# CIawevy/FreeFine

Measured on NVIDIA B200. Metric: edits/s @512^2 50-step SD1.5 (FreeFine 2-D geometric edit), higher is better.
Workload: dtype bf16

## Files before the change

### freefine_b200/csrc/attn_tcgen05.cu

```cuda
#include <cuda.h>
#include <cuda_bf16.h>

#include <atomic>
#include <cstdlib>
#include <type_traits>

#include "ff_common.cuh"

namespace {

constexpr int BM = 128;
constexpr int BN = 64;
constexpr int BOX_COLS = 64;
constexpr int TILE_BYTES = BM * 128;
constexpr int KV_BYTES = BN * 128;
constexpr int NUM_SOFTMAX_WARPS = 8;
constexpr int NUM_THREADS = 32 * (NUM_SOFTMAX_WARPS + 2);
template <bool HILO> constexpr float rescale_threshold() { return HILO ? 24.f : 8.f; }
#ifndef FF_RING_DEFAULT
#define FF_RING_DEFAULT 6
#endif
#ifndef FF_POLY_PATTERN
#define FF_POLY_PATTERN 0x92
#endif
#ifndef FF_T32_DEFAULT
#define FF_T32_DEFAULT 0
#endif
#ifndef FF_SEP_P
#define FF_SEP_P 0
#endif
#ifndef FF_SELF_ISSUE
#define FF_SELF_ISSUE 0
#endif

template <int DPAD, bool HILO> struct Cfg {
  static constexpr int DPV = DPAD == 16 ? 16 : (DPAD == 48 ? 48 : DPAD + 16);
  static constexpr int NKT = (DPAD + BOX_COLS - 1) / BOX_COLS;
  static_assert((DPV + BOX_COLS - 1) / BOX_COLS == NKT, "V tile must span as many boxes as the K tile");
  static constexpr int NSTAGE = DPAD <= 48 ? 4 : (DPAD <= 80 ? 3 : 2);
  static_assert(NSTAGE >= 2, "QK(t+1) is issued before PV(t): tile t+1 must fit beside tile t");
  static constexpr bool SEP = FF_SEP_P && DPAD == 48 && !HILO && NSTAGE == 4;
  static constexpr int TMEM_S = 0, TMEM_P = 2 * BN, TMEM_O = 2 * BN + (SEP ? BN / 2 : 0);
  static constexpr int TMEM_USED = TMEM_O + 2 * DPV;
  static constexpr int TMEM_COLS = TMEM_USED <= 256 ? 256 : 512;
  static constexpr int SMEM_Q = NKT * TILE_BYTES;
  static constexpr int SMEM_STAGE = 2 * NKT * KV_BYTES;
  static constexpr int ACC_LD = DPAD <= 80 ? DPAD + 4 : DPAD;
  static constexpr int SMEM_ACC = BM * ACC_LD * 4;
  static constexpr int SMEM_MX = 2 * BM * 4;
  static constexpr int SMEM_BYTES = SMEM_Q + NSTAGE * SMEM_STAGE + SMEM_ACC + SMEM_MX + 1024  + 256 ;
  static_assert(SMEM_BYTES <= 227 * 1024, "shared memory budget");
  static constexpr int MIN_CTAS = (SMEM_BYTES <= 113 * 1024 && TMEM_COLS == 256) ? 2 : 1;
  static constexpr bool SELF = FF_SELF_ISSUE && !SEP && DPAD == 48 && !HILO && NSTAGE == 4;
  static constexpr int THREADS = SELF ? 32 * (NUM_SOFTMAX_WARPS + 1) : NUM_THREADS;
};

__device__ __forceinline__ uint32_t smem_u32(const void* p) { return (uint32_t)__cvta_generic_to_shared(p); }

__device__ __forceinline__ void mbar_init(uint32_t bar, uint32_t count) {
  asm volatile("mbarrier.init.shared::cta.b64 [%0], %1;" ::"r"(bar), "r"(count));
}
__device__ __forceinline__ void mbar_expect_tx(uint32_t bar, uint32_t bytes) {
  asm volatile("mbarrier.arrive.expect_tx.shared::cta.b64 _, [%0], %1;" ::"r"(bar), "r"(bytes) : "memory");
}
__device__ __forceinline__ void mbar_arrive(uint32_t bar) {
  asm volatile("mbarrier.arrive.shared::cta.b64 _, [%0];" ::"r"(bar) : "memory");
}
__device__ __forceinline__ uint32_t mbar_try(uint32_t bar, uint32_t parity) {
  uint32_t done;
#ifdef FF_TRYWAIT_NOHINT
  asm volatile(
      "{\n\t.reg .pred p;\n\t"
      "mbarrier.try_wait.parity.shared::cta.b64 p, [%1], %2;\n\t"
      "selp.u32 %0, 1, 0, p;\n\t}"
      : "=r"(done)
      : "r"(bar), "r"(parity)
      : "memory");
#else
  asm volatile(
      "{\n\t.reg .pred p;\n\t"
      "mbarrier.try_wait.parity.shared::cta.b64 p, [%1], %2, %3;\n\t"
      "selp.u32 %0, 1, 0, p;\n\t}"
      : "=r"(done)
      : "r"(bar), "r"(parity), "r"(0x989680u)
      : "memory");
#endif
  return done;
}
__device__ __forceinline__ bool mbar_test(uint32_t bar, uint32_t parity) {
  uint32_t done;
  asm volatile(
      "{\n\t.reg .pred p;\n\t"
      "mbarrier.test_wait.parity.shared::cta.b64 p, [%1], %2;\n\t"
      "selp.u32 %0, 1, 0, p;\n\t}"
      : "=r"(done)
      : "r"(bar), "r"(parity)
      : "memory");
  return done != 0;
}
#ifndef FF_WAIT_FORM
#define FF_WAIT_FORM 1
#endif
__device__ __noinline__ void mbar_wait_slow(uint32_t bar, uint32_t parity) {
#if FF_WAIT_FORM == 0
  const long long t0 = clock64();
  while (!mbar_try(bar, parity)) {
    if (clock64() - t0 > 4000000000LL) {
      printf("ff_attn: mbarrier wait timed out (block %d,%d,%d thread %d bar %u parity %u)\n", blockIdx.x,
             blockIdx.y, blockIdx.z, threadIdx.x, bar, parity);
      __trap();
    }
  }
#else
  const long long t0 = clock64();
#pragma unroll 1
  for (uint32_t n = 1;; ++n) {
    if ((n & 15u) == 0 && clock64() - t0 > 4000000000LL) break;
#if FF_WAIT_FORM == 1
    if (mbar_try(bar, parity)) return;
#else
    uint32_t done;
    asm volatile(
        "{\n\t.reg .pred p;\n\t"
        "mbarrier.try_wait.parity.shared::cta.b64 p, [%1], %2;\n\t"
        "selp.u32 %0, 1, 0, p;\n\t}"
        : "=r"(done)
        : "r"(bar), "r"(parity)
        : "memory");
    if (done) return;
#endif
  }
  printf("ff_attn: mbarrier wait timed out (block %d,%d,%d thread %d bar %u parity %u)\n", blockIdx.x, blockIdx.y,
         blockIdx.z, threadIdx.x, bar, parity);
  __trap();
#endif
}
__device__ __forceinline__ void mbar_wait(uint32_t bar, uint32_t parity) {
  if (!mbar_try(bar, parity)) mbar_wait_slow(bar, parity);
}
#ifndef FF_SPIN_MASK
#define FF_SPIN_MASK 0
#endif
template <int ROLE_BIT>
__device__ __forceinline__ void mbar_wait_hot(uint32_t bar, uint32_t parity) {
  if constexpr ((FF_SPIN_MASK >> ROLE_BIT) & 1) {
    for (uint32_t n = 0; !mbar_test(bar, parity); ++n) {
#ifdef FF_SPIN_SLEEP
      __nanosleep(FF_SPIN_SLEEP);
#endif
      if (n > (1u << 24)) { mbar_wait_slow(bar, parity); return; }
    }
  } else {
    mbar_wait(bar, parity);
  }
}
__device__ __forceinline__ void tma_load_4d(uint32_t dst, const CUtensorMap* map, int c0, int c1, int c2, int c3,
                                            uint32_t bar) {
  asm volatile(
      "cp.async.bulk.tensor.4d.shared::cluster.global.tile.mbarrier::complete_tx::bytes [%0], [%1, {%2, %3, %4, %5}], [%6];"
      ::"r"(dst), "l"(map), "r"(c0), "r"(c1), "r"(c2), "r"(c3), "r"(bar)
      : "memory");
}
__device__ __forceinline__ void named_bar_sync(int id, int count) {
  switch (id) {
    case 1: asm volatile("bar.sync 1, %0;" ::"r"(count) : "memory"); break;
    case 2: asm volatile("bar.sync 2, %0;" ::"r"(count) : "memory"); break;
    case 3: asm volatile("bar.sync 3, %0;" ::"r"(count) : "memory"); break;
    default: asm volatile("bar.sync 4, %0;" ::"r"(count) : "memory"); break;
  }
}
__device__ __forceinline__ bool elect_one() {
  uint32_t pred;
  asm volatile("{\n\t.reg .pred p;\n\telect.sync _|p, 0xffffffff;\n\tselp.u32 %0, 1, 0, p;\n\t}" : "=r"(pred));
  return pred != 0;
}
__device__ __forceinline__ void tc_fence_before() { asm volatile("tcgen05.fence::before_thread_sync;" ::: "memory"); }
__device__ __forceinline__ void tc_fence_after() { asm volatile("tcgen05.fence::after_thread_sync;" ::: "memory"); }
__device__ __forceinline__ void tc_commit(uint32_t bar) {
  asm volatile("tcgen05.commit.cta_group::1.mbarrier::arrive::one.shared::cluster.b64 [%0];" ::"r"(bar) : "memory");
}
__device__ __forceinline__ void mma_ss(uint32_t d_tmem, uint64_t a_desc, uint64_t b_desc, uint32_t idesc,
                                       uint32_t accumulate) {
  asm volatile(
      "{\n\t.reg .pred p;\n\tsetp.ne.b32 p, %4, 0;\n\t"
      "tcgen05.mma.cta_group::1.kind::f16 [%0], %1, %2, %3, p;\n\t}"
      ::"r"(d_tmem), "l"(a_desc), "l"(b_desc), "r"(idesc), "r"(accumulate)
      : "memory");
}
__device__ __forceinline__ void mma_ts(uint32_t d_tmem, uint32_t a_tmem, uint64_t b_desc, uint32_t idesc,
                                       uint32_t accumulate) {
  asm volatile(
      "{\n\t.reg .pred p;\n\tsetp.ne.b32 p, %4, 0;\n\t"
      "tcgen05.mma.cta_group::1.kind::f16 [%0], [%1], %2, %3, p;\n\t}"
      ::"r"(d_tmem), "r"(a_tmem), "l"(b_desc), "r"(idesc), "r"(accumulate)
      : "memory");
}
__device__ __forceinline__ void tmem_ld32(uint32_t taddr, float (&v)[32]) {
  uint32_t* r = reinterpret_cast<uint32_t*>(v);
  asm volatile(
      "tcgen05.ld.sync.aligned.32x32b.x32.b32 "
      "{%0, %1, %2, %3, %4, %5, %6, %7, %8, %9, %10, %11, %12, %13, %14, %15, "
      "%16, %17, %18, %19, %20, %21, %22, %23, %24, %25, %26, %27, %28, %29, %30, %31}, [%32];"
      : "=r"(r[0]), "=r"(r[1]), "=r"(r[2]), "=r"(r[3]), "=r"(r[4]), "=r"(r[5]), "=r"(r[6]), "=r"(r[7]),
        "=r"(r[8]), "=r"(r[9]), "=r"(r[10]), "=r"(r[11]), "=r"(r[12]), "=r"(r[13]), "=r"(r[14]), "=r"(r[15]),
        "=r"(r[16]), "=r"(r[17]), "=r"(r[18]), "=r"(r[19]), "=r"(r[20]), "=r"(r[21]), "=r"(r[22]), "=r"(r[23]),
        "=r"(r[24]), "=r"(r[25]), "=r"(r[26]), "=r"(r[27]), "=r"(r[28]), "=r"(r[29]), "=r"(r[30]), "=r"(r[31])
      : "r"(taddr)
      : "memory");
}
__device__ __forceinline__ void tmem_ld16(uint32_t taddr, float (&v)[16]) {
  uint32_t* r = reinterpret_cast<uint32_t*>(v);
  asm volatile(
      "tcgen05.ld.sync.aligned.32x32b.x16.b32 "
      "{%0, %1, %2, %3, %4, %5, %6, %7, %8, %9, %10, %11, %12, %13, %14, %15}, [%16];"
      : "=r"(r[0]), "=r"(r[1]), "=r"(r[2]), "=r"(r[3]), "=r"(r[4]), "=r"(r[5]), "=r"(r[6]), "=r"(r[7]),
        "=r"(r[8]), "=r"(r[9]), "=r"(r[10]), "=r"(r[11]), "=r"(r[12]), "=r"(r[13]), "=r"(r[14]), "=r"(r[15])
      : "r"(taddr)
      : "memory");
}
__device__ __forceinline__ float tmem_ld1_wait(uint32_t taddr) {
  uint32_t r;
  asm volatile("tcgen05.ld.sync.aligned.32x32b.x1.b32 {%0}, [%1];\n\ttcgen05.wait::ld.sync.aligned;"
               : "=r"(r) : "r"(taddr) : "memory");
  return __uint_as_float(r);
}
__device__ __forceinline__ void tmem_st16(uint32_t taddr, const uint32_t (&r)[16]) {
  asm volatile(
      "tcgen05.st.sync.aligned.32x32b.x16.b32 [%0], "
      "{%1, %2, %3, %4, %5, %6, %7, %8, %9, %10, %11, %12, %13, %14, %15, %16};"
      ::"r"(taddr), "r"(r[0]), "r"(r[1]), "r"(r[2]), "r"(r[3]), "r"(r[4]), "r"(r[5]), "r"(r[6]), "r"(r[7]),
        "r"(r[8]), "r"(r[9]), "r"(r[10]), "r"(r[11]), "r"(r[12]), "r"(r[13]), "r"(r[14]), "r"(r[15])
      : "memory");
}
__device__ __forceinline__ void tmem_wait_ld() { asm volatile("tcgen05.wait::ld.sync.aligned;" ::: "memory"); }
__device__ __forceinline__ void tmem_wait_ld16(float (&v)[16]) {
#ifdef FF_PLAIN_WAIT
  tmem_wait_ld();
  return;
#endif
  uint32_t* r = reinterpret_cast<uint32_t*>(v);
  asm volatile("tcgen05.wait::ld.sync.aligned;"
               : "+r"(r[0]), "+r"(r[1]), "+r"(r[2]), "+r"(r[3]), "+r"(r[4]), "+r"(r[5]), "+r"(r[6]), "+r"(r[7]),
                 "+r"(r[8]), "+r"(r[9]), "+r"(r[10]), "+r"(r[11]), "+r"(r[12]), "+r"(r[13]), "+r"(r[14]), "+r"(r[15])
               :
               : "memory");
}
__device__ __forceinline__ void tmem_wait_ld32(float (&v)[32]) {
#ifdef FF_PLAIN_WAIT
  tmem_wait_ld();
  return;
#endif
  uint32_t* r = reinterpret_cast<uint32_t*>(v);
  asm volatile("tcgen05.wait::ld.sync.aligned;"
               : "+r"(r[0]), "+r"(r[1]), "+r"(r[2]), "+r"(r[3]), "+r"(r[4]), "+r"(r[5]), "+r"(r[6]), "+r"(r[7]),
                 "+r"(r[8]), "+r"(r[9]), "+r"(r[10]), "+r"(r[11]), "+r"(r[12]), "+r"(r[13]), "+r"(r[14]), "+r"(r[15]),
                 "+r"(r[16]), "+r"(r[17]), "+r"(r[18]), "+r"(r[19]), "+r"(r[20]), "+r"(r[21]), "+r"(r[22]), "+r"(r[23]),
                 "+r"(r[24]), "+r"(r[25]), "+r"(r[26]), "+r"(r[27]), "+r"(r[28]), "+r"(r[29]), "+r"(r[30]), "+r"(r[31])
               :
               : "memory");
}
__device__ __forceinline__ void tmem_wait_st() { asm volatile("tcgen05.wait::st.sync.aligned;" ::: "memory"); }
__device__ __forceinline__ float fast_exp2(float x) {
#ifdef FF_KO_MUFU
  return x;
#else
  float y;
  asm("ex2.approx.ftz.f32 %0, %1;" : "=f"(y) : "f"(x));
  return y;
#endif
}

__device__ __forceinline__ uint64_t smem_desc_sw128(uint32_t saddr, uint32_t lbo_bytes) {
  return (uint64_t)((saddr & 0x3FFFFu) >> 4) | ((uint64_t)(lbo_bytes >> 4) << 16) | ((uint64_t)(1024u >> 4) << 32) |
         (1ull << 46) | (2ull << 61);
}
__host__ __device__ constexpr uint32_t make_idesc(int n, int b_mn, bool f16 = false) {
  return (1u << 4) | (f16 ? 0u : ((1u << 7) | (1u << 10))) | ((uint32_t)b_mn << 16) | ((uint32_t)(n >> 3) << 17) |
         ((uint32_t)(BM >> 4) << 24);
}

__device__ uint32_t* g_trace = nullptr;
__device__ __forceinline__ void trace(uint32_t* tr, int role, uint32_t it, uint32_t site) {
  if (tr) {
    const uint32_t cta = blockIdx.x + gridDim.x * (blockIdx.y + gridDim.y * blockIdx.z);
    volatile uint32_t* t = tr + (size_t)cta * 8 + role * 2;
    t[0] = it;
    t[1] = site;
    __threadfence_system();
  }
}

#ifdef FF_TIMELINE
__device__ unsigned long long* g_timeline = nullptr;
#define FF_TL_TILES 64
#define FF_TL(role_, tile_, site_)                                                                      \
  do {                                                                                                  \
    if (tl && (tile_) < FF_TL_TILES) tl[(((size_t)tl_cta * 2 + (role_)) * FF_TL_TILES + (tile_)) * 8 + (site_)] = clock64(); \
  } while (0)
#else
#define FF_TL(role_, tile_, site_) do { } while (0)
#endif

struct KParams {
  const FFAttnHeadPlan* plan;
  const uint32_t* bitmasks;
  const int32_t* popc;
  void* out;
  int heads, head_dim, s_q, s_kv, mask_words, out_dtype, n_kv_streams;
  int n_streams, n_qtiles;
  float scale_log2;
};

enum { TILE_ALL = 0, TILE_IN = 1, TILE_OUT = 2, TILE_MIX = 3 };

struct SegCtx {
  int kv;
  int kmask;
  int T;
  bool kinv, prefix;
};
struct PassCtx {
  SegCtx s0, s1;
  bool rowxor, active, two_seg;
  bool has_rf0, has_rf1;
};

__device__ __forceinline__ PassCtx make_ctx(const FFAttnPass& ps, const KParams& p, int q0) {
  PassCtx c;
  c.s0.kv = ps.kv_stream;
  c.s1.kv = ps.kv_stream2;
  c.two_seg = ps.kv_stream2 >= 0;
  c.s0.kmask = ps.key_mask;
  c.s1.kmask = ps.key_mask2;
  c.s0.kinv = (ps.flags & FF_PASS_KEY_INVERT) != 0;
  c.s1.kinv = (ps.flags & FF_PASS_KEY2_INVERT) != 0;
  c.s0.prefix = (ps.flags & FF_PASS_KEY_PREFIX) != 0;
  c.s1.prefix = (ps.flags & FF_PASS_KEY2_PREFIX) != 0;
  c.s0.T = ps.key_mask >= 0 ? __ldg(p.popc + ps.key_mask) : 0;
  c.s1.T = ps.key_mask2 >= 0 ? __ldg(p.popc + ps.key_mask2) : 0;
  c.rowxor = (ps.flags & FF_PASS_ROW_XOR) != 0 && ps.row_mask >= 0;
  c.active = true;
  c.has_rf0 = true;
  c.has_rf1 = false;
  if (ps.row_mask >= 0 && (c.rowxor || (ps.flags & FF_PASS_ROW_WEIGHT))) {
    uint32_t any1 = 0, any0 = 0;
    for (int w = 0; w < BM / 32; ++w) {
      const int base = q0 + 32 * w;
      if (base >= p.s_q) break;
      const uint32_t bits = __ldg(p.bitmasks + (size_t)ps.row_mask * p.mask_words + (base >> 5));
      const int rem = p.s_q - base;
      const uint32_t valid = rem >= 32 ? 0xffffffffu : ((1u << rem) - 1u);
      any1 |= bits & valid;
      any0 |= ~bits & valid;
    }
    if (ps.flags & FF_PASS_ROW_WEIGHT) c.active = any1 != 0;
    if (c.rowxor) {
      c.has_rf0 = any0 != 0;
      c.has_rf1 = any1 != 0;
    }
  }
  return c;
}

__device__ __forceinline__ bool uniform_for(const PassCtx& c, const SegCtx& g, bool f, int s_kv) {
  if (c.two_seg || g.kmask < 0) return false;
  return (f ? s_kv - g.T : g.T) == 0;
}

__device__ __forceinline__ int tile_class(const SegCtx& g, int j, const KParams& p) {
  const int lo = j * BN;
  if (lo + BN > p.s_kv) return TILE_MIX;
  if (g.kmask < 0) return TILE_ALL;
  if (g.prefix) return lo + BN <= g.T ? TILE_IN : (lo >= g.T ? TILE_OUT : TILE_MIX);
  uint32_t a = 0xffffffffu, o = 0;
  for (int w = 0; w < BN / 32; ++w) {
    const uint32_t bits = __ldg(p.bitmasks + (size_t)g.kmask * p.mask_words + (lo >> 5) + w);
    a &= bits;
    o |= bits;
  }
  return a == 0xffffffffu ? TILE_IN : (o == 0 ? TILE_OUT : TILE_MIX);
}

__device__ __forceinline__ int run_end(const SegCtx& g, int j, int cls, const KParams& p) {
  if (cls == TILE_MIX || (g.kmask >= 0 && !g.prefix)) return j + 1;
  const int n_full = p.s_kv / BN;
  if (cls == TILE_IN) { const int t = g.T / BN; return t < n_full ? t : n_full; }
  return n_full;
}

__device__ __forceinline__ bool row_allowed(int cls, bool flip, bool uniform) {
  return uniform || cls == TILE_ALL || ((cls == TILE_IN) != flip);
}

__device__ __forceinline__ bool tile_skip(const PassCtx& c, const SegCtx& g, int cls, int s_kv) {
  if (cls == TILE_MIX || cls == TILE_ALL) return false;
  bool need = false;
  if (c.has_rf0) need = need || row_allowed(cls, g.kinv, uniform_for(c, g, g.kinv, s_kv));
  if (c.has_rf1) need = need || row_allowed(cls, !g.kinv, uniform_for(c, g, !g.kinv, s_kv));
  return !need;
}

__device__ __forceinline__ uint32_t pack_bf16x2(float lo, float hi) {
  const __nv_bfloat162 b = __floats2bfloat162_rn(lo, hi);
  return *reinterpret_cast<const uint32_t*>(&b);
}

template <bool MASKED>
__device__ __forceinline__ void softmax_chunk_hilo(const float* s, uint32_t* hl, float sc, float nb, uint32_t bits) {
  const float2 sc2 = make_float2(sc, sc), nb2 = make_float2(nb, nb);
#pragma unroll
  for (int i = 0; i < 8; ++i) {
    float2 x = __ffma2_rn(make_float2(s[2 * i], s[2 * i + 1]), sc2, nb2);
    if (MASKED) {
      x.x = (bits >> (2 * i)) & 1u ? x.x : -INFINITY;
      x.y = (bits >> (2 * i + 1)) & 1u ? x.y : -INFINITY;
    }
    const float2 e = make_float2(fast_exp2(x.x), fast_exp2(x.y));
    const uint32_t b0 = __float_as_uint(e.x), b1 = __float_as_uint(e.y);
    hl[i] = __byte_perm(b0, b1, 0x7632);
    const float2 r = __fadd2_rn(e, make_float2(-__uint_as_float(b0 & 0xffff0000u), -__uint_as_float(b1 & 0xffff0000u)));
    hl[8 + i] = pack_bf16x2(r.x, r.y);
  }
}

__device__ __forceinline__ float2 poly_exp2_x2(float2 x) {
  const float MAGIC = 12582912.f;
  x.x = fmaxf(x.x, -125.f);
  x.y = fmaxf(x.y, -125.f);
  const float2 t = __fadd2_rn(x, make_float2(MAGIC, MAGIC));
  const float2 n = __fadd2_rn(t, make_float2(-MAGIC, -MAGIC));
  const float2 f = __fadd2_rn(x, make_float2(-n.x, -n.y));
  float2 r = __ffma2_rn(make_float2(0.055205512791872025f, 0.055205512791872025f), f,
                        make_float2(0.24261389672756195f, 0.24261389672756195f));
  r = __ffma2_rn(r, f, make_float2(0.6932547688484192f, 0.6932547688484192f));
  r = __ffma2_rn(r, f, make_float2(0.9999276995658875f, 0.9999276995658875f));
  r.x = __int_as_float(__float_as_int(r.x) + (__float_as_int(t.x) << 23));
  r.y = __int_as_float(__float_as_int(r.y) + (__float_as_int(t.y) << 23));
  return r;
}

__device__ __forceinline__ uint32_t pack_f16x2(float lo, float hi) {
  uint32_t r;
  asm("cvt.rn.f16x2.f32 %0, %1, %2;" : "=r"(r) : "f"(hi), "f"(lo));
  return r;
}

template <bool MASKED>
__device__ __forceinline__ void softmax_chunk_f16(const float* s, uint32_t* pk, float sc, float nb, uint32_t bits) {
  const float2 sc2 = make_float2(sc, sc), nb2 = make_float2(nb, nb);
#pragma unroll
  for (int i = 0; i < 8; ++i) {
    float2 x = __ffma2_rn(make_float2(s[2 * i], s[2 * i + 1]), sc2, nb2);
    float2 e;
    if (MASKED) {
      x.x = (bits >> (2 * i)) & 1u ? x.x : -INFINITY;
      x.y = (bits >> (2 * i + 1)) & 1u ? x.y : -INFINITY;
      e = make_float2(fast_exp2(x.x), fast_exp2(x.y));
#ifdef FF_KO_EXP
    } else if (true) {
      e = x;
#endif
    } else if ((FF_POLY_PATTERN >> i) & 1) {
      e = poly_exp2_x2(x);
    } else {
      e = make_float2(fast_exp2(x.x), fast_exp2(x.y));
    }
    pk[i] = pack_f16x2(e.x, e.y);
  }
}


#ifndef FF_LEAN_ISSUER
#define FF_LEAN_ISSUER 1
#endif
__device__ __forceinline__ void lean_wait(uint32_t bar, uint32_t parity) {
  uint32_t done;
  asm volatile(
      "{\n\t.reg .pred p;\n\t"
      "mbarrier.try_wait.parity.shared::cta.b64 p, [%1], %2;\n\t"
      "selp.u32 %0, 1, 0, p;\n\t}"
      : "=r"(done)
      : "r"(bar), "r"(parity)
      : "memory");
#ifdef FF_LEAN_SPIN
  for (int n = 0; !done && n < FF_LEAN_SPIN; ++n) done = mbar_test(bar, parity);
#endif
  if (!done) mbar_wait_slow(bar, parity);
}
__device__ __forceinline__ void lean_qk48(uint32_t sbuf, uint64_t qdesc, uint64_t kdesc, uint32_t idesc, uint32_t bar_s_) {
  asm volatile(
      "{\n\t.reg .pred e, pf, pt;\n\t.reg .b64 q1, q2, k1, k2;\n\t"
      "elect.sync _|e, 0xffffffff;\n\t"
      "setp.ne.b32 pf, 0, 0;\n\tsetp.eq.b32 pt, 0, 0;\n\t"
      "add.u64 q1, %1, 2;\n\tadd.u64 q2, %1, 4;\n\tadd.u64 k1, %2, 2;\n\tadd.u64 k2, %2, 4;\n\t"
      "@e tcgen05.mma.cta_group::1.kind::f16 [%0], %1, %2, %3, pf;\n\t"
      "@e tcgen05.mma.cta_group::1.kind::f16 [%0], q1, k1, %3, pt;\n\t"
      "@e tcgen05.mma.cta_group::1.kind::f16 [%0], q2, k2, %3, pt;\n\t"
      "@e tcgen05.commit.cta_group::1.mbarrier::arrive::one.shared::cluster.b64 [%4];\n\t}"
      ::"r"(sbuf), "l"(qdesc), "l"(kdesc), "r"(idesc), "r"(bar_s_)
      : "memory");
}
#ifdef FF_KO_PV1
#define FF_KO_PVSTEPS(x)
#else
#define FF_KO_PVSTEPS(x) x
#endif
#ifdef FF_KO_QK1
#define FF_KO_QKSTEPS(x)
#else
#define FF_KO_QKSTEPS(x) x
#endif
template <bool WITH_QK>
__device__ __forceinline__ void lean_pv_qk48(uint32_t obuf, uint32_t sp, uint64_t vdesc, uint32_t idesc_pv, uint32_t acc0,
                                             uint32_t bar_kve, uint64_t qdesc, uint64_t kdesc, uint32_t idesc_qk,
                                             uint32_t bar_s_) {
  if constexpr (WITH_QK) {
    asm volatile(
        "{\n\t.reg .pred e, p0, pf, pt;\n\t.reg .b64 v1, v2, v3, q1, q2, k1, k2;\n\t.reg .b32 a1, a2, a3;\n\t"
        "elect.sync _|e, 0xffffffff;\n\t"
        "setp.ne.b32 p0, %4, 0;\n\tsetp.ne.b32 pf, 0, 0;\n\tsetp.eq.b32 pt, 0, 0;\n\t"
        "add.u64 v1, %2, 128;\n\tadd.u64 v2, %2, 256;\n\tadd.u64 v3, %2, 384;\n\t"
        "add.u32 a1, %1, 8;\n\tadd.u32 a2, %1, 32;\n\tadd.u32 a3, %1, 40;\n\t"
        "add.u64 q1, %6, 2;\n\tadd.u64 q2, %6, 4;\n\tadd.u64 k1, %7, 2;\n\tadd.u64 k2, %7, 4;\n\t"
        "@e tcgen05.mma.cta_group::1.kind::f16 [%0], [%1], %2, %3, p0;\n\t"
        FF_KO_PVSTEPS("@e tcgen05.mma.cta_group::1.kind::f16 [%0], [a1], v1, %3, pt;\n\t")
        FF_KO_PVSTEPS("@e tcgen05.mma.cta_group::1.kind::f16 [%0], [a2], v2, %3, pt;\n\t")
        FF_KO_PVSTEPS("@e tcgen05.mma.cta_group::1.kind::f16 [%0], [a3], v3, %3, pt;\n\t")
        "@e tcgen05.commit.cta_group::1.mbarrier::arrive::one.shared::cluster.b64 [%5];\n\t"
        "@e tcgen05.mma.cta_group::1.kind::f16 [%1], %6, %7, %8, pf;\n\t"
        FF_KO_QKSTEPS("@e tcgen05.mma.cta_group::1.kind::f16 [%1], q1, k1, %8, pt;\n\t")
        FF_KO_QKSTEPS("@e tcgen05.mma.cta_group::1.kind::f16 [%1], q2, k2, %8, pt;\n\t")
        "@e tcgen05.commit.cta_group::1.mbarrier::arrive::one.shared::cluster.b64 [%9];\n\t}"
        ::"r"(obuf), "r"(sp), "l"(vdesc), "r"(idesc_pv), "r"(acc0), "r"(bar_kve), "l"(qdesc), "l"(kdesc), "r"(idesc_qk),
          "r"(bar_s_)
        : "memory");
  } else {
    asm volatile(
        "{\n\t.reg .pred e, p0, pt;\n\t.reg .b64 v1, v2, v3;\n\t.reg .b32 a1, a2, a3;\n\t"
        "elect.sync _|e, 0xffffffff;\n\t"
        "setp.ne.b32 p0, %4, 0;\n\tsetp.eq.b32 pt, 0, 0;\n\t"
        "add.u64 v1, %2, 128;\n\tadd.u64 v2, %2, 256;\n\tadd.u64 v3, %2, 384;\n\t"
        "add.u32 a1, %1, 8;\n\tadd.u32 a2, %1, 32;\n\tadd.u32 a3, %1, 40;\n\t"
        "@e tcgen05.mma.cta_group::1.kind::f16 [%0], [%1], %2, %3, p0;\n\t"
        "@e tcgen05.mma.cta_group::1.kind::f16 [%0], [a1], v1, %3, pt;\n\t"
        "@e tcgen05.mma.cta_group::1.kind::f16 [%0], [a2], v2, %3, pt;\n\t"
        "@e tcgen05.mma.cta_group::1.kind::f16 [%0], [a3], v3, %3, pt;\n\t"
        "@e tcgen05.commit.cta_group::1.mbarrier::arrive::one.shared::cluster.b64 [%5];\n\t"
        "@e tcgen05.commit.cta_group::1.mbarrier::arrive::one.shared::cluster.b64 [%6];\n\t}"
        ::"r"(obuf), "r"(sp), "l"(vdesc), "r"(idesc_pv), "r"(acc0), "r"(bar_kve), "r"(bar_s_)
        : "memory");
  }
}

__device__ __forceinline__ void lean_pv48_sep(uint32_t obuf, uint32_t pbase, uint64_t vdesc, uint32_t idesc_pv, uint32_t acc0,
                                              uint32_t bar_kve, uint32_t bar_o_) {
  asm volatile(
      "{\n\t.reg .pred e, p0, pt;\n\t.reg .b64 v1, v2, v3;\n\t.reg .b32 a1, a2, a3;\n\t"
      "elect.sync _|e, 0xffffffff;\n\t"
      "setp.ne.b32 p0, %4, 0;\n\tsetp.eq.b32 pt, 0, 0;\n\t"
      "add.u64 v1, %2, 128;\n\tadd.u64 v2, %2, 256;\n\tadd.u64 v3, %2, 384;\n\t"
      "add.u32 a1, %1, 8;\n\tadd.u32 a2, %1, 16;\n\tadd.u32 a3, %1, 24;\n\t"
      "@e tcgen05.mma.cta_group::1.kind::f16 [%0], [%1], %2, %3, p0;\n\t"
      "@e tcgen05.mma.cta_group::1.kind::f16 [%0], [a1], v1, %3, pt;\n\t"
      "@e tcgen05.mma.cta_group::1.kind::f16 [%0], [a2], v2, %3, pt;\n\t"
      "@e tcgen05.mma.cta_group::1.kind::f16 [%0], [a3], v3, %3, pt;\n\t"
      "@e tcgen05.commit.cta_group::1.mbarrier::arrive::one.shared::cluster.b64 [%5];\n\t"
      "@e tcgen05.commit.cta_group::1.mbarrier::arrive::one.shared::cluster.b64 [%6];\n\t}"
      ::"r"(obuf), "r"(pbase), "l"(vdesc), "r"(idesc_pv), "r"(acc0), "r"(bar_kve), "r"(bar_o_)
      : "memory");
}

template <int DPAD, bool P_HILO>
__global__ void __launch_bounds__(Cfg<DPAD, P_HILO>::THREADS, Cfg<DPAD, P_HILO>::MIN_CTAS)
attn_masked_kv_kernel(const __grid_constant__ CUtensorMap tm_q, const __grid_constant__ CUtensorMap tm_k,
                      const __grid_constant__ CUtensorMap tm_v, const KParams p) {
  using C = Cfg<DPAD, P_HILO>;
  extern __shared__ uint8_t smem_raw[];
  const uint32_t smem_base = (smem_u32(smem_raw) + 1023u) & ~1023u;
  const uint32_t sQ = smem_base;
  const uint32_t sKV = smem_base + C::SMEM_Q;
  const uint32_t sACC = sKV + C::NSTAGE * C::SMEM_STAGE;
  const uint32_t sMX = sACC + C::SMEM_ACC;
  const uint32_t bar_base = sMX + C::SMEM_MX;
  const uint32_t bar_q = bar_base;
  const uint32_t bar_s = bar_base + 16, bar_p = bar_base + 32;
  const uint32_t bar_kv_full = bar_base + 48, bar_kv_empty = bar_base + 48 + 8 * C::NSTAGE;
  const uint32_t tmem_slot = bar_base + 48 + 16 * C::NSTAGE;
  const uint32_t bar_f = bar_base + 192, bar_o = bar_base + 208;
  static_assert(48 + 16 * C::NSTAGE + 8 <= 192, "barrier block layout");
  uint8_t* gen_base = smem_raw + (smem_base - smem_u32(smem_raw));
  float* const acc_smem = reinterpret_cast<float*>(gen_base + (sACC - smem_base));
  float* const mx_smem = reinterpret_cast<float*>(gen_base + (sMX - smem_base));
  volatile uint32_t* tmem_slot_ptr =
      reinterpret_cast<volatile uint32_t*>(gen_base + (tmem_slot - smem_base));

  const int warp = threadIdx.x >> 5, lane = threadIdx.x & 31;
  const int q0 = blockIdx.x * BM, head = blockIdx.y, stream = blockIdx.z;
  const FFAttnHeadPlan* plan = p.plan + (size_t)stream * p.heads + head;
  int n_pass = __ldg(&plan->n_pass);
  n_pass = n_pass < 0 ? 0 : (n_pass > FF_MAX_PASS ? FF_MAX_PASS : n_pass);
  const int n_kv_tiles = (p.s_kv + BN - 1) / BN;

  if (threadIdx.x == 0) {
    mbar_init(bar_q, 1);
    mbar_init(bar_s, 1);
    mbar_init(bar_s + 8, 1);
    mbar_init(bar_p, NUM_SOFTMAX_WARPS / 2);
    mbar_init(bar_p + 8, NUM_SOFTMAX_WARPS / 2);
    mbar_init(bar_f, NUM_SOFTMAX_WARPS / 2);
    mbar_init(bar_f + 8, NUM_SOFTMAX_WARPS / 2);
    mbar_init(bar_o, 1);
    mbar_init(bar_o + 8, 1);
    for (int i = 0; i < C::NSTAGE; ++i) {
      mbar_init(bar_kv_full + 8 * i, 1);
      mbar_init(bar_kv_empty + 8 * i, 1);
    }
    asm volatile("fence.mbarrier_init.release.cluster;" ::: "memory");
  }
  if (warp == NUM_SOFTMAX_WARPS) {
    asm volatile("tcgen05.alloc.cta_group::1.sync.aligned.shared::cta.b32 [%0], %1;" ::"r"(tmem_slot),
                 "r"((uint32_t)C::TMEM_COLS)
                 : "memory");
    asm volatile("tcgen05.relinquish_alloc_permit.cta_group::1.sync.aligned;" ::: "memory");
  }
  tc_fence_before();
  __syncthreads();
  tc_fence_after();
  const uint32_t tmem = *tmem_slot_ptr;
#ifdef FF_ENABLE_TRACE
  uint32_t* const tr = g_trace;
  const int trole = warp == NUM_SOFTMAX_WARPS ? 0 : (warp == NUM_SOFTMAX_WARPS + 1 ? 1 : (threadIdx.x == 0 ? 2 : (threadIdx.x == 32 * NUM_SOFTMAX_WARPS - 32 ? 3 : -1)));
#define FF_TRACE(it_, site_) do { if (tr && trole >= 0 && (warp < NUM_SOFTMAX_WARPS || lane == 0)) trace(tr, trole, (uint32_t)(it_), (site_)); } while (0)
#else
#define FF_TRACE(it_, site_) do { } while (0)
#endif
  FF_TRACE(0, 1);
#ifdef FF_TIMELINE
  const int tl_lin = blockIdx.x + gridDim.x * (blockIdx.y + gridDim.y * blockIdx.z);
  const int tl_cta = tl_lin == 4000 ? 0 : 1;
  unsigned long long* const tl = ((tl_lin == 4000 || tl_lin == 4101) && lane == 0 &&
                                  (warp == 0 || warp == NUM_SOFTMAX_WARPS + 1)) ? g_timeline : nullptr;
#endif

  if (warp == NUM_SOFTMAX_WARPS) {
    if (lane == 0) {
      mbar_expect_tx(bar_q, C::NKT * TILE_BYTES);
      for (int kt = 0; kt < C::NKT; ++kt)
        tma_load_4d(sQ + kt * TILE_BYTES, &tm_q, kt * BOX_COLS, head, q0, stream, bar_q);
      int it = 0;
#pragma unroll 1
      for (int ip = 0; ip < n_pass; ++ip) {
        const FFAttnPass ps = plan->pass[ip];
        const PassCtx cx = make_ctx(ps, p, q0);
        if (!cx.active) continue;
#pragma unroll 1
        for (int seg = 0; seg < 2; ++seg) {
          const SegCtx sg = seg ? cx.s1 : cx.s0;
          if (sg.kv < 0) continue;
#pragma unroll 1
          for (int j0 = 0; j0 < n_kv_tiles;) {
            const int cls = tile_class(sg, j0, p), j1 = run_end(sg, j0, cls, p), jb = j0;
            j0 = j1;
            if (tile_skip(cx, sg, cls, p.s_kv)) continue;
#pragma unroll 1
            for (int j = jb; j < j1; ++j) {
            const int stage = it % C::NSTAGE, use = it / C::NSTAGE;
            FF_TRACE(it, 10);
            if (use > 0) mbar_wait_hot<2>(bar_kv_empty + 8 * stage, (use - 1) & 1);
            FF_TRACE(it, 11);
            const uint32_t full = bar_kv_full + 8 * stage;
            const uint32_t sK = sKV + stage * C::SMEM_STAGE, sV = sK + C::NKT * KV_BYTES;
#ifdef FF_KO_TMA
            if (it >= C::NSTAGE) { mbar_arrive(full); ++it; continue; }
#endif
            mbar_expect_tx(full, 2 * C::NKT * KV_BYTES);
            for (int kt = 0; kt < C::NKT; ++kt) {
              tma_load_4d(sK + kt * KV_BYTES, &tm_k, kt * BOX_COLS, head, j * BN, sg.kv, full);
              tma_load_4d(sV + kt * KV_BYTES, &tm_v, kt * BOX_COLS, head, j * BN, sg.kv, full);
            }
            ++it;
            }
          }
        }
      }
    }
  } else if (!C::SELF && warp == NUM_SOFTMAX_WARPS + 1) {
    {
      const bool leader = elect_one();
      constexpr uint32_t idesc_qk = make_idesc(BN, 0);
      constexpr uint32_t idesc_pv = make_idesc(C::DPV, 1, !P_HILO);
      const uint64_t qdesc0 = smem_desc_sw128(sQ, 16);
      const uint64_t kdesc0 = smem_desc_sw128(sKV, 16);
      const uint64_t vdesc0 = smem_desc_sw128(sKV + C::NKT * KV_BYTES, KV_BYTES);
      int pe0 = 0, pe1 = 0, pe2 = 0, n_total = 0;
#pragma unroll
      for (int ip = 0; ip < FF_MAX_PASS; ++ip) {
        if (ip < n_pass) {
          const FFAttnPass ps = plan->pass[ip];
          const PassCtx cx = make_ctx(ps, p, q0);
          if (cx.active) {
#pragma unroll 1
            for (int seg = 0; seg < 2; ++seg) {
              const SegCtx sg = seg ? cx.s1 : cx.s0;
              if (sg.kv < 0) continue;
#pragma unroll 1
              for (int j0 = 0; j0 < n_kv_tiles;) {
                const int cls = tile_class(sg, j0, p), j1 = run_end(sg, j0, cls, p), jb = j0;
                j0 = j1;
                if (!tile_skip(cx, sg, cls, p.s_kv)) n_total += j1 - jb;
              }
            }
          }
        }
        if (ip == 0) pe0 = n_total;
        if (ip == 1) pe1 = n_total;
        if (ip == 2) pe2 = n_total;
      }
      FF_TRACE(0, 20);
      mbar_wait(bar_q, 0);
      if constexpr (C::SEP) {
        tc_fence_after();
        if (n_total > 0) { lean_wait(bar_kv_full, 0); tc_fence_after(); lean_qk48(tmem + C::TMEM_S, qdesc0, kdesc0, idesc_qk, bar_s); }
        if (n_total > 1) {
          lean_wait(bar_kv_full + 8, 0);
          tc_fence_after();
          lean_qk48(tmem + C::TMEM_S + BN, qdesc0, kdesc0 + (uint64_t)(C::SMEM_STAGE >> 4), idesc_qk, bar_s + 8);
        }
        uint32_t gph = 0;
        int t = 0;
#pragma unroll 1
        while (t < n_total) {
#pragma unroll
          for (int u = 0; u < 4; ++u) {
            if (t < n_total) {
              const int pstart = t >= pe2 ? pe2 : (t >= pe1 ? pe1 : (t >= pe0 ? pe0 : 0));
              const uint32_t acc0 = (t - pstart < 2) ? 0u : 1u;
              FF_TL(1, t, 0);
              if (t + 2 < n_total) {
                lean_wait(bar_kv_full + 8 * ((u + 2) & 3), u < 2 ? gph : gph ^ 1u);
                lean_wait(bar_f + 8 * (u & 1), (uint32_t)((u >> 1) & 1));
                FF_TL(1, t, 1);
                tc_fence_after();
                lean_qk48(tmem + C::TMEM_S + BN * (u & 1), qdesc0, kdesc0 + (uint64_t)((((u + 2) & 3) * C::SMEM_STAGE) >> 4),
                          idesc_qk, bar_s + 8 * (u & 1));
              }
              FF_TL(1, t, 2);
              lean_wait(bar_p, (uint32_t)(u & 1));
              FF_TL(1, t, 3);
              tc_fence_after();
              lean_pv48_sep(tmem + C::TMEM_O + C::DPV * (u & 1), tmem + C::TMEM_P, vdesc0 + (uint64_t)((u * C::SMEM_STAGE) >> 4),
                            idesc_pv, acc0, bar_kv_empty + 8 * u, bar_o + 8 * (u & 1));
              FF_TL(1, t, 4);
              ++t;
            }
          }
          gph ^= 1u;
        }
        __syncwarp();
      } else if constexpr (FF_LEAN_ISSUER && DPAD == 48 && !P_HILO && C::NSTAGE == 4) {
        tc_fence_after();
        if (n_total > 0) { lean_wait(bar_kv_full, 0); tc_fence_after(); lean_qk48(tmem + C::TMEM_S, qdesc0, kdesc0, idesc_qk, bar_s); }
        if (n_total > 1) {
          lean_wait(bar_kv_full + 8, 0);
          tc_fence_after();
          lean_qk48(tmem + C::TMEM_S + BN, qdesc0, kdesc0 + (uint64_t)(C::SMEM_STAGE >> 4), idesc_qk, bar_s + 8);
        }
        uint32_t gph = 0;
        int t = 0;
#pragma unroll 1
        while (t < n_total) {
#pragma unroll
          for (int u = 0; u < 4; ++u) {
            if (t < n_total) {
              const bool more = t + 2 < n_total;
              const int pstart = t >= pe2 ? pe2 : (t >= pe1 ? pe1 : (t >= pe0 ? pe0 : 0));
              const uint32_t acc0 = (t - pstart < 2) ? 0u : 1u;
              const uint32_t sp = tmem + C::TMEM_S + BN * (u & 1);
              const uint32_t obuf = tmem + C::TMEM_O + C::DPV * (u & 1);
              const uint64_t vd = vdesc0 + (uint64_t)((u * C::SMEM_STAGE) >> 4);
              const uint64_t kd = kdesc0 + (uint64_t)((((u + 2) & 3) * C::SMEM_STAGE) >> 4);
              if (more) lean_wait(bar_kv_full + 8 * ((u + 2) & 3), u < 2 ? gph : gph ^ 1u);
              lean_wait(bar_p + 8 * (u & 1), (uint32_t)((u >> 1) & 1));
              tc_fence_after();
              if (more) lean_pv_qk48<true>(obuf, sp, vd, idesc_pv, acc0, bar_kv_empty + 8 * u, qdesc0, kd, idesc_qk, bar_s + 8 * (u & 1));
              else lean_pv_qk48<false>(obuf, sp, vd, idesc_pv, acc0, bar_kv_empty + 8 * u, 0, 0, 0, bar_s + 8 * (u & 1));
              ++t;
            }
          }
          gph ^= 1u;
        }
        __syncwarp();
      } else {
      int qk_t = 0;
      uint32_t q_stage = 0, q_phase = 0, p_stage = 0;
      auto wait_kv = [&]() { mbar_wait_hot<1>(bar_kv_full + 8 * q_stage, q_phase); };
      auto issue_qk = [&]() {
        const uint64_t kd = kdesc0 + ((q_stage * (uint32_t)C::SMEM_STAGE) >> 4);
        const uint32_t sbuf = tmem + C::TMEM_S + BN * (qk_t & 1);
#pragma unroll
        for (int ks = 0; ks < DPAD / 16; ++ks) {
          const uint32_t qoff = (ks >> 2) * TILE_BYTES + (ks & 3) * 32;
          const uint32_t koff = (ks >> 2) * KV_BYTES + (ks & 3) * 32;
          mma_ss(sbuf, qdesc0 + (qoff >> 4), kd + (koff >> 4), idesc_qk, ks > 0);
        }
        tc_commit(bar_s + 8 * (qk_t & 1));
      };
      auto advance_qk = [&]() {
        ++qk_t;
        if (++q_stage == (uint32_t)C::NSTAGE) { q_stage = 0; q_phase ^= 1u; }
      };
#pragma unroll 1
      for (int k = 0; k < 2 && qk_t < n_total; ++k) {
        wait_kv();
        tc_fence_after();
        if (leader) issue_qk();
        __syncwarp();
        advance_qk();
      }
#pragma unroll 1
      for (int t = 0; t < n_total; ++t) {
        const bool more = qk_t < n_total;
        const int pstart = t >= pe2 ? pe2 : (t >= pe1 ? pe1 : (t >= pe0 ? pe0 : 0));
        const bool first_of_parity = t - pstart < 2;
        const uint64_t vd = vdesc0 + ((p_stage * (uint32_t)C::SMEM_STAGE) >> 4);
        const uint32_t pbase = tmem + C::TMEM_S + BN * (t & 1);
        const uint32_t obuf = tmem + C::TMEM_O + C::DPV * (t & 1);
        bool kv_ready = more && __all_sync(0xffffffffu, mbar_test(bar_kv_full + 8 * q_stage, q_phase));
        FF_TL(1, t, 0);
        mbar_wait_hot<1>(bar_p + 8 * (t & 1), (t >> 1) & 1);
        FF_TL(1, t, 3);
        if (more && !kv_ready) kv_ready = __all_sync(0xffffffffu, mbar_test(bar_kv_full + 8 * q_stage, q_phase));
        tc_fence_after();
        if (leader) {
#pragma unroll
          for (int ks = 0; ks < BN / 16; ++ks) {
            const uint64_t vdesc = vd + ((ks * 2048) >> 4);
            if constexpr (P_HILO) {
              mma_ts(obuf, pbase + 16 * ks, vdesc, idesc_pv, (!first_of_parity || ks > 0) ? 1u : 0u);
              mma_ts(obuf, pbase + 16 * ks + 8, vdesc, idesc_pv, 1u);
            } else {
              mma_ts(obuf, pbase + 32 * (ks >> 1) + 8 * (ks & 1), vdesc, idesc_pv,
                     (!first_of_parity || ks > 0) ? 1u : 0u);
            }
          }
          tc_commit(bar_kv_empty + 8 * p_stage);
          if (kv_ready) issue_qk();
          else if (!more) tc_commit(bar_s + 8 * (t & 1));
        }
        __syncwarp();
        if (more && !kv_ready) {
          wait_kv();
          tc_fence_after();
          if (leader) issue_qk();
          __syncwarp();
        }
        if (more) advance_qk();
        FF_TL(1, t, 4);
        if (++p_stage == (uint32_t)C::NSTAGE) p_stage = 0;
      }
      __syncwarp();
      }
    }
  } else {
    const int wq = warp & 3;
    const int wg = warp >> 2;
    const int rloc = 32 * wq + lane;
    const int row = q0 + rloc;
    const uint32_t tlane = tmem + ((uint32_t)(wq * 32) << 16);
    const uint32_t tS = tlane + C::TMEM_S + BN * wg;
    const uint32_t tO = tlane + C::TMEM_O + C::DPV * wg;
    const uint32_t tOx = tlane + C::TMEM_O + C::DPV * (wg ^ 1);
    float* const acc_row = acc_smem + (size_t)rloc * C::ACC_LD;
    bool acc_started = false;
    int it = 0;
    int n_total = 0;
    [[maybe_unused]] constexpr uint32_t s_idesc_qk = make_idesc(BN, 0);
    [[maybe_unused]] constexpr uint32_t s_idesc_pv = make_idesc(C::DPV, 1, !P_HILO);
    [[maybe_unused]] const uint64_t s_qdesc0 = smem_desc_sw128(sQ, 16);
    [[maybe_unused]] const uint64_t s_kdesc0 = smem_desc_sw128(sKV, 16);
    [[maybe_unused]] const uint64_t s_vdesc0 = smem_desc_sw128(sKV + C::NKT * KV_BYTES, KV_BYTES);
    if constexpr (C::SELF) {
      if (wq == 0) {
#pragma unroll 1
        for (int ip = 0; ip < n_pass; ++ip) {
          const FFAttnPass ps = plan->pass[ip];
          const PassCtx cx = make_ctx(ps, p, q0);
          if (!cx.active) continue;
#pragma unroll 1
          for (int seg = 0; seg < 2; ++seg) {
            const SegCtx sg = seg ? cx.s1 : cx.s0;
            if (sg.kv < 0) continue;
#pragma unroll 1
            for (int j0 = 0; j0 < n_kv_tiles;) {
              const int cls = tile_class(sg, j0, p), j1 = run_end(sg, j0, cls, p), jb = j0;
              j0 = j1;
              if (!tile_skip(cx, sg, cls, p.s_kv)) n_total += j1 - jb;
            }
          }
        }
        n_total = __shfl_sync(0xffffffffu, n_total, 0);
        if (wg < n_total) {
          mbar_wait(bar_q, 0);
          lean_wait(bar_kv_full + 8 * wg, 0);
          tc_fence_after();
          lean_qk48(tmem + C::TMEM_S + BN * wg, s_qdesc0, s_kdesc0 + (uint64_t)((wg * C::SMEM_STAGE) >> 4), s_idesc_qk,
                    bar_s + 8 * wg);
        }
      }
    }
#pragma unroll 1
    for (int ip = 0; ip < n_pass; ++ip) {
      const FFAttnPass ps = plan->pass[ip];
      const PassCtx cx = make_ctx(ps, p, q0);
      if (!cx.active) continue;
      uint32_t rb = 0;
      if (ps.row_mask >= 0 && row < p.s_q)
        rb = (__ldg(p.bitmasks + (size_t)ps.row_mask * p.mask_words + (row >> 5)) >> (row & 31)) & 1u;
      const bool rowflip = cx.rowxor && rb;
      float m_used = -INFINITY;
      int n_mine = 0, last_mine = 0;
      const int it_pass0 = it;
#pragma unroll 1
      for (int seg = 0; seg < 2; ++seg) {
        const SegCtx sg = seg ? cx.s1 : cx.s0;
        if (sg.kv < 0) continue;
        const bool flip = sg.kinv != rowflip;
        const bool uniform = uniform_for(cx, sg, flip, p.s_kv);
        const float sc = uniform ? 0.f : p.scale_log2;
#pragma unroll 1
        for (int j0 = 0; j0 < n_kv_tiles;) {
          const int cls = tile_class(sg, j0, p), j1 = run_end(sg, j0, cls, p), jb = j0;
          j0 = j1;
          if (tile_skip(cx, sg, cls, p.s_kv)) continue;
          const bool row_ok_cls = row_allowed(cls, flip, uniform);
          int j = jb + (((it ^ wg) & 1) ? 1 : 0);
          int itj = it + (j - jb);
          it += j1 - jb;
#pragma unroll 1
          for (; j < j1; j += 2, itj += 2) {
            FF_TRACE(itj, 30);
            FF_TL(0, itj, 0);
            mbar_wait_hot<0>(bar_s + 8 * wg, (itj >> 1) & 1);
            FF_TL(0, itj, 1);
            FF_TRACE(itj, 31);
            tc_fence_after();
            uint32_t kb_lo = 0xffffffffu, kb_hi = 0xffffffffu;
            if (cls == TILE_MIX) {
#pragma unroll
              for (int w = 0; w < 2; ++w) {
                const int kbase = j * BN + 32 * w;
                const int rem = p.s_kv - kbase;
                const uint32_t valid = rem >= 32 ? 0xffffffffu : (rem <= 0 ? 0u : ((1u << rem) - 1u));
                uint32_t kb = 0xffffffffu;
                if (sg.kmask >= 0 && !uniform && rem > 0) {
                  if (sg.prefix) {
                    const int t = sg.T - kbase;
                    kb = t >= 32 ? 0xffffffffu : (t <= 0 ? 0u : ((1u << t) - 1u));
                  } else {
                    kb = __ldg(p.bitmasks + (size_t)sg.kmask * p.mask_words + (kbase >> 5));
                  }
                  if (flip) kb = ~kb;
                }
                if (w == 0) kb_lo = kb & valid; else kb_hi = kb & valid;
              }
            }
            float mt, sb[32];
            {
              float sa[32];
              tmem_ld32(tS, sa);
#ifdef FF_LD_BOTH
              tmem_ld32(tS + 32, sb);
#endif
              tmem_wait_ld32(sa);
              float m0, m1;
              if (cls != TILE_MIX) {
                m0 = fmaxf(sa[0], sa[1]);
                m1 = fmaxf(sa[2], sa[3]);
#pragma unroll
                for (int i = 4; i < 32; i += 4) {
                  m0 = fmaxf(m0, fmaxf(sa[i], sa[i + 1]));
                  m1 = fmaxf(m1, fmaxf(sa[i + 2], sa[i + 3]));
                }
              } else {
                m0 = m1 = -INFINITY;
#pragma unroll
                for (int i = 0; i < 32; i += 2) {
                  m0 = fmaxf(m0, (kb_lo >> i) & 1u ? sa[i] : -INFINITY);
                  m1 = fmaxf(m1, (kb_lo >> (i + 1)) & 1u ? sa[i + 1] : -INFINITY);
                }
              }
              mt = fmaxf(m0, m1);
            }
            {
#ifdef FF_KO_LD2
#pragma unroll
              for (int i = 0; i < 32; ++i) sb[i] = mt + (float)i;
#else
#ifndef FF_LD_BOTH
              tmem_ld32(tS + 32, sb);
#endif
              tmem_wait_ld32(sb);
#endif
              float m0, m1;
              if (cls != TILE_MIX) {
                m0 = fmaxf(sb[0], sb[1]);
                m1 = fmaxf(sb[2], sb[3]);
#pragma unroll
                for (int i = 4; i < 32; i += 4) {
                  m0 = fmaxf(m0, fmaxf(sb[i], sb[i + 1]));
                  m1 = fmaxf(m1, fmaxf(sb[i + 2], sb[i + 3]));
                }
              } else {
                m0 = m1 = -INFINITY;
#pragma unroll
                for (int i = 0; i < 32; i += 2) {
                  m0 = fmaxf(m0, (kb_hi >> i) & 1u ? sb[i] : -INFINITY);
                  m1 = fmaxf(m1, (kb_hi >> (i + 1)) & 1u ? sb[i + 1] : -INFINITY);
                }
              }
              mt = fmaxf(mt, fmaxf(m0, m1));
              if (cls != TILE_MIX && !row_ok_cls) mt = -INFINITY;
#ifdef FF_KO_MAX
              mt = 0.f;
#endif
            }
            FF_TL(0, itj, 2);
            const float mts = uniform ? 0.f : mt * p.scale_log2;
            float alpha = 1.f;
            bool grow = false;
            if (n_mine == 0) {
              m_used = mts;
            } else if (mts > m_used + rescale_threshold<P_HILO>()) {
              alpha = fast_exp2(m_used - mts);
              m_used = mts;
              grow = true;
            }
            const bool any_grow = __any_sync(0xffffffffu, grow);
            auto rescale_o = [&]() {
#pragma unroll
              for (int c = 0; c < C::DPV / 16; ++c) {
                float o[16];
                uint32_t ob[16];
                tmem_ld16(tO + 16 * c, o);
                tmem_wait_ld16(o);
#pragma unroll
                for (int i = 0; i < 16; ++i) ob[i] = __float_as_uint(o[i] * alpha);
                tmem_st16(tO + 16 * c, ob);
              }
            };
            if (!C::SEP && any_grow) rescale_o();
            FF_TL(0, itj, 3);
            const float nb = (cls == TILE_MIX || row_ok_cls) ? -m_used : -INFINITY;
            uint32_t pk[(P_HILO || C::SEP) ? 32 : 16];
#pragma unroll
            for (int hb = 1; hb >= 0; --hb) {
              float sa[32];
#ifdef FF_KO_REREAD
              const float* sv = sb;
#else
              if (hb == 0) {
                tmem_ld32(tS, sa);
                tmem_wait_ld32(sa);
                if constexpr (C::SEP) {
                  tc_fence_before();
                  __syncwarp();
                  if (lane == 0) mbar_arrive(bar_f + 8 * wg);
                }
              }
              const float* sv = hb ? sb : sa;
#endif
              const uint32_t kbits = hb ? kb_hi : kb_lo;
              if (cls != TILE_MIX) {
#pragma unroll
                for (int jj = 0; jj < 2; ++jj) {
                  if constexpr (P_HILO) softmax_chunk_hilo<false>(sv + 16 * jj, pk + 16 * jj, sc, nb, 0u);
                  else softmax_chunk_f16<false>(sv + 16 * jj, pk + (C::SEP ? 16 * hb : 0) + 8 * jj, sc, nb, 0u);
                }
              } else {
#pragma unroll
                for (int jj = 0; jj < 2; ++jj) {
                  const uint32_t bits = (kbits >> (16 * jj)) & 0xffffu;
                  if constexpr (P_HILO) softmax_chunk_hilo<true>(sv + 16 * jj, pk + 16 * jj, sc, nb, bits);
                  else softmax_chunk_f16<true>(sv + 16 * jj, pk + (C::SEP ? 16 * hb : 0) + 8 * jj, sc, nb, bits);
                }
              }
              if constexpr (P_HILO) {
                tmem_st16(tS + 32 * hb, *reinterpret_cast<const uint32_t(*)[16]>(pk));
                tmem_st16(tS + 32 * hb + 16, *reinterpret_cast<const uint32_t(*)[16]>(pk + 16));
              } else if constexpr (!C::SEP) {
                tmem_st16(tS + 32 * hb, *reinterpret_cast<const uint32_t(*)[16]>(pk));
              }
            }
            if constexpr (C::SEP) {
              if (itj >= 1) {
                const uint32_t bo = bar_o + 8 * (wg ^ 1), po = (uint32_t)(((itj - 1) >> 1) & 1);
                if (!mbar_test(bo, po)) mbar_wait(bo, po);
              }
              tc_fence_after();
              if (any_grow) rescale_o();
              tmem_st16(tlane + C::TMEM_P, *reinterpret_cast<const uint32_t(*)[16]>(pk));
              tmem_st16(tlane + C::TMEM_P + 16, *reinterpret_cast<const uint32_t(*)[16]>(pk + 16));
            }
            FF_TL(0, itj, 4);
            tmem_wait_st();
            FF_TL(0, itj, 5);
            tc_fence_before();
            if constexpr (C::SELF) {
              named_bar_sync(3 + wg, 128);
              if (wq == 0) {
                const int stg = itj & 3, nxt = (itj + 2) & 3;
                const bool more = itj + 2 < n_total;
                if (more) lean_wait(bar_kv_full + 8 * nxt, (uint32_t)(((itj + 2) >> 2) & 1));
                tc_fence_after();
                const uint32_t sp = tmem + C::TMEM_S + BN * wg;
                const uint32_t obuf = tmem + C::TMEM_O + C::DPV * wg;
                const uint64_t vd = s_vdesc0 + (uint64_t)((stg * C::SMEM_STAGE) >> 4);
                const uint64_t kd = s_kdesc0 + (uint64_t)((nxt * C::SMEM_STAGE) >> 4);
                const uint32_t acc0 = n_mine == 0 ? 0u : 1u;
                if (more) lean_pv_qk48<true>(obuf, sp, vd, s_idesc_pv, acc0, bar_kv_empty + 8 * stg, s_qdesc0, kd, s_idesc_qk, bar_s + 8 * wg);
                else lean_pv_qk48<false>(obuf, sp, vd, s_idesc_pv, acc0, bar_kv_empty + 8 * stg, 0, 0, 0, bar_s + 8 * wg);
              }
            } else {
              __syncwarp();
              if (lane == 0) mbar_arrive(C::SEP ? bar_p : bar_p + 8 * wg);
            }
            FF_TL(0, itj, 6);
            FF_TRACE(itj, 34);
            ++n_mine;
            last_mine = itj;
          }
        }
      }
      if (it == it_pass0) continue;
      FF_TRACE(it, 35);
      if constexpr (C::SEP) {
        const int L = it - 1;
        mbar_wait(bar_o + 8 * (L & 1), (uint32_t)((L >> 1) & 1));
        tc_fence_after();
      } else if (n_mine > 0) mbar_wait_hot<0>(bar_s + 8 * wg, ((last_mine + 2) >> 1) & 1);
      FF_TRACE(it, 36);
      mx_smem[wg * BM + rloc] = n_mine > 0 ? m_used : -INFINITY;
      tc_fence_before();
      named_bar_sync(1, 32 * NUM_SOFTMAX_WARPS);
      tc_fence_after();
      const float m_other = mx_smem[(wg ^ 1) * BM + rloc];
      const float m_all = fmaxf(m_used, m_other);
      const bool wrote_mine = n_mine > 0, wrote_other = (it - it_pass0) - n_mine > 0;
      const float a_mine = (wrote_mine && m_used > -INFINITY) ? fast_exp2(m_used - m_all) : 0.f;
      const float a_other = (wrote_other && m_other > -INFINITY) ? fast_exp2(m_other - m_all) : 0.f;
      float l = 0.f;
      if (wrote_mine) l = a_mine * tmem_ld1_wait(tO + p.head_dim);
      if (wrote_other) l = fmaf(a_other, tmem_ld1_wait(tOx + p.head_dim), l);
      float coef = ps.weight;
      if (ps.flags & FF_PASS_ROW_WEIGHT) coef = rb ? coef : 0.f;
      coef = l > 0.f ? coef / l : 0.f;
      const float c_mine = coef * a_mine, c_other = coef * a_other;
#pragma unroll
      for (int c = 0; c < DPAD / 16; ++c) {
        if ((c & 1) != wg) continue;
        float r[16];
#pragma unroll
        for (int i = 0; i < 16; ++i) r[i] = acc_started ? acc_row[16 * c + i] : 0.f;
        if (wrote_mine) {
          float o[16];
          tmem_ld16(tO + 16 * c, o);
          tmem_wait_ld16(o);
#pragma unroll
          for (int i = 0; i < 16; ++i) r[i] = fmaf(c_mine, o[i], r[i]);
        }
        if (wrote_other) {
          float o[16];
          tmem_ld16(tOx + 16 * c, o);
          tmem_wait_ld16(o);
#pragma unroll
          for (int i = 0; i < 16; ++i) r[i] = fmaf(c_other, o[i], r[i]);
        }
#pragma unroll
        for (int i = 0; i < 16; i += 4)
          *reinterpret_cast<float4*>(acc_row + 16 * c + i) = make_float4(r[i], r[i + 1], r[i + 2], r[i + 3]);
      }
      acc_started = true;
      tc_fence_before();
      named_bar_sync(2, 32 * NUM_SOFTMAX_WARPS);
      tc_fence_after();
    }
    {
      const bool row_ok = row < p.s_q;
      const size_t o_off = ((size_t)stream * p.s_q + (row_ok ? row : 0)) * ((size_t)p.heads * p.head_dim) +
                           (size_t)head * p.head_dim;
#pragma unroll
      for (int c = 0; c < DPAD / 16; ++c) {
        if ((c & 1) != wg) continue;
        float o[16];
#pragma unroll
        for (int i = 0; i < 16; ++i) o[i] = acc_started ? acc_row[16 * c + i] : 0.f;
#pragma unroll
        for (int g = 0; g < 2; ++g) {
          if (row_ok && 16 * c + 8 * g < p.head_dim) {
            if (p.out_dtype == FF_DT_BF16) {
              uint4 v;
              v.x = pack_bf16x2(o[8 * g + 0], o[8 * g + 1]);
              v.y = pack_bf16x2(o[8 * g + 2], o[8 * g + 3]);
              v.z = pack_bf16x2(o[8 * g + 4], o[8 * g + 5]);
              v.w = pack_bf16x2(o[8 * g + 6], o[8 * g + 7]);
              *reinterpret_cast<uint4*>(static_cast<__nv_bfloat16*>(p.out) + o_off + 16 * c + 8 * g) = v;
            } else {
              float4* dst = reinterpret_cast<float4*>(static_cast<float*>(p.out) + o_off + 16 * c + 8 * g);
              dst[0] = make_float4(o[8 * g + 0], o[8 * g + 1], o[8 * g + 2], o[8 * g + 3]);
              dst[1] = make_float4(o[8 * g + 4], o[8 * g + 5], o[8 * g + 6], o[8 * g + 7]);
            }
          }
        }
      }
    }
  }
  FF_TRACE(0, 90);
  tc_fence_before();
  __syncthreads();
  if (warp == NUM_SOFTMAX_WARPS) {
    tc_fence_after();
    asm volatile("tcgen05.dealloc.cta_group::1.sync.aligned.b32 %0, %1;" ::"r"(tmem), "r"((uint32_t)C::TMEM_COLS)
                 : "memory");
  }
}

#include "attn_ring.cuh"
#include "attn_t32.cuh"

typedef CUresult (*EncodeTiledFn)(CUtensorMap*, CUtensorMapDataType, cuuint32_t, void*, const cuuint64_t*,
                                  const cuuint64_t*, const cuuint32_t*, const cuuint32_t*, CUtensorMapInterleave,
                                  CUtensorMapSwizzle, CUtensorMapL2promotion, CUtensorMapFloatOOBfill);

EncodeTiledFn get_encode_fn() {
  static EncodeTiledFn fn = nullptr;
  if (!fn) {
    void* ptr = nullptr;
    cudaDriverEntryPointQueryResult qres;
    if (cudaGetDriverEntryPoint("cuTensorMapEncodeTiled", &ptr, cudaEnableDefault, &qres) == cudaSuccess &&
        qres == cudaDriverEntryPointSuccess)
      fn = reinterpret_cast<EncodeTiledFn>(ptr);
  }
  return fn;
}

int make_map(CUtensorMap* map, const void* base, int streams, int S, int heads, int d, int box_rows,
             bool f16 = false) {
  EncodeTiledFn enc = get_encode_fn();
  if (!enc) return ff::fail(FF_E_CUDA, "cuTensorMapEncodeTiled entry point not found");
  const cuuint64_t C = (cuuint64_t)heads * d;
  cuuint64_t dims[4] = {(cuuint64_t)d, (cuuint64_t)heads, (cuuint64_t)S, (cuuint64_t)streams};
  cuuint64_t strides[3] = {(cuuint64_t)d * 2, C * 2, (cuuint64_t)S * C * 2};
  cuuint32_t box[4] = {BOX_COLS, 1, (cuuint32_t)box_rows, 1};
  cuuint32_t estr[4] = {1, 1, 1, 1};
  CUresult r = enc(map, f16 ? CU_TENSOR_MAP_DATA_TYPE_FLOAT16 : CU_TENSOR_MAP_DATA_TYPE_BFLOAT16, 4, const_cast<void*>(base), dims, strides, box, estr,
                   CU_TENSOR_MAP_INTERLEAVE_NONE, CU_TENSOR_MAP_SWIZZLE_128B, CU_TENSOR_MAP_L2_PROMOTION_L2_128B,
                   CU_TENSOR_MAP_FLOAT_OOB_FILL_NONE);
  if (r != CUDA_SUCCESS)
    return ff::fail(FF_E_CUDA, "cuTensorMapEncodeTiled failed (CUresult %d) dims=[%d,%d,%d,%d]", (int)r, d, heads, S,
                    streams);
  return FF_OK;
}

template <typename K>
int ensure_smem(K kernel, int bytes, std::atomic<uint64_t>& done) {
  int dev = 0;
  cudaGetDevice(&dev);
  const uint64_t bit = 1ull << (dev & 63);
  if (done.load(std::memory_order_acquire) & bit) return FF_OK;
  cudaError_t e = cudaFuncSetAttribute(kernel, cudaFuncAttributeMaxDynamicSharedMemorySize, bytes);
  if (e != cudaSuccess) return ff::fail(FF_E_CUDA, "cudaFuncSetAttribute(smem=%d): %s", bytes, cudaGetErrorString(e));
  done.fetch_or(bit, std::memory_order_release);
  return FF_OK;
}

template <int DPAD, bool HILO>
int launch(const CUtensorMap& mq, const CUtensorMap& mk, const CUtensorMap& mv, const KParams& kp, int n_streams,
           cudaStream_t st) {
  using C = Cfg<DPAD, HILO>;
  static std::atomic<uint64_t> configured{0};
  int rc = ensure_smem(attn_masked_kv_kernel<DPAD, HILO>, C::SMEM_BYTES, configured);
  if (rc != FF_OK) return rc;
  dim3 grid((kp.s_q + BM - 1) / BM, kp.heads, n_streams);
  attn_masked_kv_kernel<DPAD, HILO><<<grid, C::THREADS, C::SMEM_BYTES, st>>>(mq, mk, mv, kp);
  return ff::check_launch("ff_attn_masked_kv");
}

int sm_count() {
  static std::atomic<int> cached[64];
  int dev = 0;
  cudaGetDevice(&dev);
  int n = cached[dev & 63].load(std::memory_order_relaxed);
  if (n == 0) {
    cudaDeviceGetAttribute(&n, cudaDevAttrMultiProcessorCount, dev);
    if (n <= 0) n = 148;
    cached[dev & 63].store(n, std::memory_order_relaxed);
  }
  return n;
}

template <int DPAD, int NWG, int NBUF, bool TOKEN>
int launch_ring(const CUtensorMap& mq, const CUtensorMap& mk, const CUtensorMap& mv, const KParams& kp, int n_streams,
                cudaStream_t st) {
  using C = RCfg<DPAD, NWG, NBUF>;
  static std::atomic<uint64_t> configured{0};
  int rc = ensure_smem(attn_ring_kernel<DPAD, NWG, NBUF, TOKEN>, C::SMEM_BYTES, configured);
  if (rc != FF_OK) return rc;
  const int n_items = kp.n_qtiles * kp.heads * n_streams;
  int ctas = sm_count() * C::MIN_CTAS;
  if (ctas > n_items) ctas = n_items;
  attn_ring_kernel<DPAD, NWG, NBUF, TOKEN><<<ctas, C::NUM_THREADS, C::SMEM_BYTES, st>>>(mq, mk, mv, kp);
  return ff::check_launch("ff_attn_masked_kv (ring kernel)");
}

int launch_t32(const CUtensorMap& mq, const CUtensorMap& mk, const CUtensorMap& mv, const KParams& kp, int n_streams, cudaStream_t st) {
  static std::atomic<uint64_t> configured{0};
  int rc = ensure_smem(attn_t32_kernel, T32::SMEM_BYTES, configured);
  if (rc != FF_OK) return rc;
  dim3 grid((kp.s_q + BM - 1) / BM, kp.heads, n_streams);
  attn_t32_kernel<<<grid, NUM_THREADS, T32::SMEM_BYTES, st>>>(mq, mk, mv, kp);
  return ff::check_launch("ff_attn_masked_kv (32-key tiles)");
}

int t32_mode() {
  static int mode = -1;
  if (mode < 0) {
    const char* e = getenv("FF_ATTN_T32");
    mode = e ? (atoi(e) != 0) : FF_T32_DEFAULT;
  }
  return mode;
}

int ring_mode() {
  static int mode = -1;
  if (mode < 0) {
    const char* e = getenv("FF_ATTN_RING");
    mode = e ? atoi(e) : FF_RING_DEFAULT;
    if (mode < 0 || mode > 7) mode = FF_RING_DEFAULT;
  }
  return mode;
}

}

extern "C" int ff_debug_set_timeline(void* device_ptr) {
#ifdef FF_TIMELINE
  cudaError_t e = cudaMemcpyToSymbol(g_timeline, &device_ptr, sizeof(void*));
  if (e != cudaSuccess) return ff::fail(FF_E_CUDA, "ff_debug_set_timeline: %s", cudaGetErrorString(e));
  return FF_OK;
#else
  (void)device_ptr;
  return ff::fail(FF_E_UNSUPPORTED, "ff_debug_set_timeline: library built without -DFF_TIMELINE");
#endif
}

extern "C" int ff_debug_set_trace(void* device_visible_ptr) {
#ifndef FF_ENABLE_TRACE
  if (device_visible_ptr) return ff::fail(FF_E_UNSUPPORTED, "ff_debug_set_trace: library built without FF_TRACE=1");
#endif
  cudaError_t e = cudaMemcpyToSymbol(g_trace, &device_visible_ptr, sizeof(void*));
  if (e != cudaSuccess) return ff::fail(FF_E_CUDA, "ff_debug_set_trace: %s", cudaGetErrorString(e));
  return FF_OK;
}

extern "C" int ff_attn_v_head_stride(int32_t head_dim) {
  if (head_dim <= 8) return Cfg<16, false>::DPV;
  if (head_dim <= 40) return Cfg<48, false>::DPV;
  if (head_dim <= 80) return Cfg<80, false>::DPV;
  return Cfg<160, false>::DPV;
}

extern "C" int ff_attn_masked_kv(const FFAttnArgs* a, void* stream) {
  FF_REQUIRE(a != nullptr, "ff_attn_masked_kv: null args");
  FF_REQUIRE(a->q && a->k && a->v && a->out && a->plan, "ff_attn_masked_kv: null pointer");
  FF_REQUIRE(a->n_streams > 0 && a->n_kv_streams > 0 && a->heads > 0 && a->s_q > 0 && a->s_kv > 0,
             "ff_attn_masked_kv: bad shape");
  FF_REQUIRE(a->head_dim >= 8 && a->head_dim % 8 == 0, "ff_attn_masked_kv: head_dim=%d must be a multiple of 8",
             a->head_dim);
  if (a->head_dim > 160) return ff::fail(FF_E_UNSUPPORTED, "ff_attn_masked_kv: head_dim=%d > 160", a->head_dim);
  FF_REQUIRE(a->heads <= 65535 && a->n_streams <= 65535, "ff_attn_masked_kv: heads / streams exceed grid limits");
  FF_REQUIRE(ff::aligned16(a->q) && ff::aligned16(a->k) && ff::aligned16(a->v) && ff::aligned16(a->out),
             "ff_attn_masked_kv: q/k/v/out must be 16-byte aligned");
  FF_REQUIRE(a->out_dtype == FF_DT_BF16 || a->out_dtype == FF_DT_F32, "ff_attn_masked_kv: bad out_dtype");
  FF_REQUIRE(a->v_dtype == FF_DT_BF16 || a->v_dtype == FF_DT_F16, "ff_attn_masked_kv: v_dtype must be bf16 or f16");
  FF_REQUIRE(a->scale > 0.f, "ff_attn_masked_kv: scale must be positive");
  if (a->n_masks > 0) {
    FF_REQUIRE(a->bitmasks && a->mask_popcount, "ff_attn_masked_kv: n_masks>0 but no bitmasks / popcounts");
    const int need = ((a->s_q > a->s_kv ? a->s_q : a->s_kv) + 31) / 32;
    FF_REQUIRE(a->mask_words >= need, "ff_attn_masked_kv: mask_words=%d < %d", a->mask_words, need);
  }
  int dev = 0, major = 0;
  cudaGetDevice(&dev);
  {
    static std::atomic<int> cached_major[64];
    major = cached_major[dev & 63].load(std::memory_order_relaxed);
    if (major == 0) {
      cudaDeviceGetAttribute(&major, cudaDevAttrComputeCapabilityMajor, dev);
      cached_major[dev & 63].store(major, std::memory_order_relaxed);
    }
  }
  if (major != 10) return ff::fail(FF_E_ARCH, "ff_attn_masked_kv: needs an sm_100 device (got sm_%d*)", major);

  alignas(64) CUtensorMap mq, mk, mv;
  int rc;
  if ((rc = make_map(&mq, a->q, a->n_streams, a->s_q, a->heads, a->head_dim, BM)) != FF_OK) return rc;
  const bool v_f16 = a->v_dtype == FF_DT_F16;
  const bool use_t32 = v_f16 && a->head_dim > 8 && a->head_dim <= 40 && t32_mode() != 0;
  const int kv_rows = use_t32 ? TBN : BN;
  if ((rc = make_map(&mk, a->k, a->n_kv_streams, a->s_kv, a->heads, a->head_dim, kv_rows)) != FF_OK) return rc;
  FF_REQUIRE(a->v_head_stride == ff_attn_v_head_stride(a->head_dim),
             "ff_attn_masked_kv: V must be staged by ff_kv_gather_cast (v_head_stride=%d, expected %d)",
             a->v_head_stride, ff_attn_v_head_stride(a->head_dim));
  if ((rc = make_map(&mv, a->v, a->n_kv_streams, a->s_kv, a->heads, a->v_head_stride, kv_rows, v_f16)) != FF_OK) return rc;

  KParams kp;
  kp.plan = a->plan;
  kp.bitmasks = a->bitmasks;
  kp.popc = a->mask_popcount;
  kp.out = a->out;
  kp.heads = a->heads;
  kp.head_dim = a->head_dim;
  kp.s_q = a->s_q;
  kp.s_kv = a->s_kv;
  kp.mask_words = a->mask_words;
  kp.out_dtype = a->out_dtype;
  kp.n_kv_streams = a->n_kv_streams;
  kp.n_streams = a->n_streams;
  kp.n_qtiles = (a->s_q + BM - 1) / BM;
  kp.scale_log2 = a->scale * 1.4426950408889634f;
  cudaStream_t st = static_cast<cudaStream_t>(stream);
  const int d = a->head_dim;
  if (v_f16) {
    if (d <= 8) return launch<16, false>(mq, mk, mv, kp, a->n_streams, st);
    if (use_t32) return launch_t32(mq, mk, mv, kp, a->n_streams, st);
    const int rm = ring_mode();
    if (rm == 1 && d <= 40) return launch_ring<48, 1, 3, false>(mq, mk, mv, kp, a->n_streams, st);
    if (rm == 2 && d <= 40) return launch_ring<48, 2, 4, false>(mq, mk, mv, kp, a->n_streams, st);
    if (rm == 3 && d <= 40) return launch_ring<48, 3, 5, false>(mq, mk, mv, kp, a->n_streams, st);
    if (rm == 7 && d <= 40) return launch_ring<48, 4, 5, false>(mq, mk, mv, kp, a->n_streams, st);
    if (rm == 4 && d <= 40) return launch_ring<48, 3, 5, true>(mq, mk, mv, kp, a->n_streams, st);
    if (rm == 5 && d <= 40) return launch_ring<48, 2, 4, true>(mq, mk, mv, kp, a->n_streams, st);
    if (d > 40 && d <= 80 && (rm == 4 || rm == 5)) return launch_ring<80, 2, 3, true>(mq, mk, mv, kp, a->n_streams, st);
    if (d > 40 && d <= 80 && rm != 0) return launch_ring<80, 2, 3, false>(mq, mk, mv, kp, a->n_streams, st);
    if (d <= 40) return launch<48, false>(mq, mk, mv, kp, a->n_streams, st);
    if (d <= 80) return launch<80, false>(mq, mk, mv, kp, a->n_streams, st);
    return launch<160, false>(mq, mk, mv, kp, a->n_streams, st);
  }
  if (d <= 8) return launch<16, true>(mq, mk, mv, kp, a->n_streams, st);
  if (d <= 40) return launch<48, true>(mq, mk, mv, kp, a->n_streams, st);
  if (d <= 80) return launch<80, true>(mq, mk, mv, kp, a->n_streams, st);
  return launch<160, true>(mq, mk, mv, kp, a->n_streams, st);
}
```

Measured before the change: 2.776.

## Route first half of P to a dedicated TMEM slot so QK(t+2) overlaps softmax

After: 2.801, median of 6. No clear change (+0.9%).

```diff
diff --git a/freefine_b200/csrc/attn_tcgen05.cu b/freefine_b200/csrc/attn_tcgen05.cu
--- a/freefine_b200/csrc/attn_tcgen05.cu
+++ b/freefine_b200/csrc/attn_tcgen05.cu
@@ -1,5 +1,6 @@
 #include <cuda.h>
 #include <cuda_bf16.h>
+#include <cuda_fp16.h>
 
 #include <atomic>
 #include <cstdlib>
@@ -26,12 +27,6 @@
 #ifndef FF_T32_DEFAULT
 #define FF_T32_DEFAULT 0
 #endif
-#ifndef FF_SEP_P
-#define FF_SEP_P 0
-#endif
-#ifndef FF_SELF_ISSUE
-#define FF_SELF_ISSUE 0
-#endif
 
 template <int DPAD, bool HILO> struct Cfg {
   static constexpr int DPV = DPAD == 16 ? 16 : (DPAD == 48 ? 48 : DPAD + 16);
@@ -39,9 +34,9 @@
   static_assert((DPV + BOX_COLS - 1) / BOX_COLS == NKT, "V tile must span as many boxes as the K tile");
   static constexpr int NSTAGE = DPAD <= 48 ? 4 : (DPAD <= 80 ? 3 : 2);
   static_assert(NSTAGE >= 2, "QK(t+1) is issued before PV(t): tile t+1 must fit beside tile t");
-  static constexpr bool SEP = FF_SEP_P && DPAD == 48 && !HILO && NSTAGE == 4;
-  static constexpr int TMEM_S = 0, TMEM_P = 2 * BN, TMEM_O = 2 * BN + (SEP ? BN / 2 : 0);
-  static constexpr int TMEM_USED = TMEM_O + 2 * DPV;
+  static constexpr bool LAZY = DPAD == 48 && !HILO && NSTAGE == 4;
+  static constexpr int TMEM_S = 0, TMEM_O = 2 * BN, TMEM_P = TMEM_O + 2 * DPV;
+  static constexpr int TMEM_USED = TMEM_P + (LAZY ? BN / 2 : 0);
   static constexpr int TMEM_COLS = TMEM_USED <= 256 ? 256 : 512;
   static constexpr int SMEM_Q = NKT * TILE_BYTES;
   static constexpr int SMEM_STAGE = 2 * NKT * KV_BYTES;
@@ -51,8 +46,6 @@
   static constexpr int SMEM_BYTES = SMEM_Q + NSTAGE * SMEM_STAGE + SMEM_ACC + SMEM_MX + 1024  + 256 ;
   static_assert(SMEM_BYTES <= 227 * 1024, "shared memory budget");
   static constexpr int MIN_CTAS = (SMEM_BYTES <= 113 * 1024 && TMEM_COLS == 256) ? 2 : 1;
-  static constexpr bool SELF = FF_SELF_ISSUE && !SEP && DPAD == 48 && !HILO && NSTAGE == 4;
-  static constexpr int THREADS = SELF ? 32 * (NUM_SOFTMAX_WARPS + 1) : NUM_THREADS;
 };
 
 __device__ __forceinline__ uint32_t smem_u32(const void* p) { return (uint32_t)__cvta_generic_to_shared(p); }
@@ -470,6 +463,45 @@
 }
 
 
+__device__ __forceinline__ float max16(const float* s, bool mix, uint32_t kb) {
+  float m0, m1;
+  if (!mix) {
+    m0 = fmaxf(s[0], s[1]);
+    m1 = fmaxf(s[2], s[3]);
+#pragma unroll
+    for (int i = 4; i < 16; i += 4) {
+      m0 = fmaxf(m0, fmaxf(s[i], s[i + 1]));
+      m1 = fmaxf(m1, fmaxf(s[i + 2], s[i + 3]));
+    }
+  } else {
+    m0 = m1 = -INFINITY;
+#pragma unroll
+    for (int i = 0; i < 16; i += 2) {
+      m0 = fmaxf(m0, (kb >> i) & 1u ? s[i] : -INFINITY);
+      m1 = fmaxf(m1, (kb >> (i + 1)) & 1u ? s[i + 1] : -INFINITY);
+    }
+  }
+  return fmaxf(m0, m1);
+}
+__device__ __forceinline__ float max32(const float (&s)[32], bool mix, uint32_t kb) {
+  return fmaxf(max16(s, mix, kb), max16(s + 16, mix, kb >> 16));
+}
+__device__ __forceinline__ void exp32_f16(const float (&s)[32], uint32_t* pk, bool mix, uint32_t kb, float sc, float nb) {
+  if (!mix) {
+    softmax_chunk_f16<false>(s, pk, sc, nb, 0u);
+    softmax_chunk_f16<false>(s + 16, pk + 8, sc, nb, 0u);
+  } else {
+    softmax_chunk_f16<true>(s, pk, sc, nb, kb & 0xffffu);
+    softmax_chunk_f16<true>(s + 16, pk + 8, sc, nb, kb >> 16);
+  }
+}
+__device__ __forceinline__ uint32_t pmax16(const uint32_t* pk) {
+  __half2 m = *reinterpret_cast<const __half2*>(pk);
+#pragma unroll
+  for (int i = 1; i < 16; ++i) m = __hmax2(m, *reinterpret_cast<const __half2*>(pk + i));
+  const uint32_t u = *reinterpret_cast<const uint32_t*>(&m);
+  return max(u & 0xffffu, u >> 16);
+}
 #ifndef FF_LEAN_ISSUER
 #define FF_LEAN_ISSUER 1
 #endif
@@ -511,67 +543,49 @@
 #define FF_KO_QKSTEPS(x) x
 #endif
 template <bool WITH_QK>
-__device__ __forceinline__ void lean_pv_qk48(uint32_t obuf, uint32_t sp, uint64_t vdesc, uint32_t idesc_pv, uint32_t acc0,
-                                             uint32_t bar_kve, uint64_t qdesc, uint64_t kdesc, uint32_t idesc_qk,
-                                             uint32_t bar_s_) {
+__device__ __forceinline__ void lean_pv_qk48(uint32_t obuf, uint32_t pp, uint32_t sp, uint64_t vdesc, uint32_t idesc_pv,
+                                             uint32_t acc0, uint32_t bar_kve, uint64_t qdesc, uint64_t kdesc,
+                                             uint32_t idesc_qk, uint32_t bar_s_) {
   if constexpr (WITH_QK) {
     asm volatile(
         "{\n\t.reg .pred e, p0, pf, pt;\n\t.reg .b64 v1, v2, v3, q1, q2, k1, k2;\n\t.reg .b32 a1, a2, a3;\n\t"
         "elect.sync _|e, 0xffffffff;\n\t"
-        "setp.ne.b32 p0, %4, 0;\n\tsetp.ne.b32 pf, 0, 0;\n\tsetp.eq.b32 pt, 0, 0;\n\t"
-        "add.u64 v1, %2, 128;\n\tadd.u64 v2, %2, 256;\n\tadd.u64 v3, %2, 384;\n\t"
-        "add.u32 a1, %1, 8;\n\tadd.u32 a2, %1, 32;\n\tadd.u32 a3, %1, 40;\n\t"
-        "add.u64 q1, %6, 2;\n\tadd.u64 q2, %6, 4;\n\tadd.u64 k1, %7, 2;\n\tadd.u64 k2, %7, 4;\n\t"
-        "@e tcgen05.mma.cta_group::1.kind::f16 [%0], [%1], %2, %3, p0;\n\t"
-        FF_KO_PVSTEPS("@e tcgen05.mma.cta_group::1.kind::f16 [%0], [a1], v1, %3, pt;\n\t")
-        FF_KO_PVSTEPS("@e tcgen05.mma.cta_group::1.kind::f16 [%0], [a2], v2, %3, pt;\n\t")
-        FF_KO_PVSTEPS("@e tcgen05.mma.cta_group::1.kind::f16 [%0], [a3], v3, %3, pt;\n\t")
-        "@e tcgen05.commit.cta_group::1.mbarrier::arrive::one.shared::cluster.b64 [%5];\n\t"
-        "@e tcgen05.mma.cta_group::1.kind::f16 [%1], %6, %7, %8, pf;\n\t"
-        FF_KO_QKSTEPS("@e tcgen05.mma.cta_group::1.kind::f16 [%1], q1, k1, %8, pt;\n\t")
-        FF_KO_QKSTEPS("@e tcgen05.mma.cta_group::1.kind::f16 [%1], q2, k2, %8, pt;\n\t")
-        "@e tcgen05.commit.cta_group::1.mbarrier::arrive::one.shared::cluster.b64 [%9];\n\t}"
-        ::"r"(obuf), "r"(sp), "l"(vdesc), "r"(idesc_pv), "r"(acc0), "r"(bar_kve), "l"(qdesc), "l"(kdesc), "r"(idesc_qk),
-          "r"(bar_s_)
+        "setp.ne.b32 p0, %5, 0;\n\tsetp.ne.b32 pf, 0, 0;\n\tsetp.eq.b32 pt, 0, 0;\n\t"
+        "add.u64 v1, %3, 128;\n\tadd.u64 v2, %3, 256;\n\tadd.u64 v3, %3, 384;\n\t"
+        "add.u32 a1, %1, 8;\n\tadd.u32 a2, %2, 32;\n\tadd.u32 a3, %2, 40;\n\t"
+        "add.u64 q1, %7, 2;\n\tadd.u64 q2, %7, 4;\n\tadd.u64 k1, %8, 2;\n\tadd.u64 k2, %8, 4;\n\t"
+        "@e tcgen05.mma.cta_group::1.kind::f16 [%0], [%1], %3, %4, p0;\n\t"
+        FF_KO_PVSTEPS("@e tcgen05.mma.cta_group::1.kind::f16 [%0], [a1], v1, %4, pt;\n\t")
+        FF_KO_PVSTEPS("@e tcgen05.mma.cta_group::1.kind::f16 [%0], [a2], v2, %4, pt;\n\t")
+        FF_KO_PVSTEPS("@e tcgen05.mma.cta_group::1.kind::f16 [%0], [a3], v3, %4, pt;\n\t")
+        "@e tcgen05.commit.cta_group::1.mbarrier::arrive::one.shared::cluster.b64 [%6];\n\t"
+        "@e tcgen05.mma.cta_group::1.kind::f16 [%2], %7, %8, %9, pf;\n\t"
+        FF_KO_QKSTEPS("@e tcgen05.mma.cta_group::1.kind::f16 [%2], q1, k1, %9, pt;\n\t")
+        FF_KO_QKSTEPS("@e tcgen05.mma.cta_group::1.kind::f16 [%2], q2, k2, %9, pt;\n\t")
+        "@e tcgen05.commit.cta_group::1.mbarrier::arrive::one.shared::cluster.b64 [%10];\n\t}"
+        ::"r"(obuf), "r"(pp), "r"(sp), "l"(vdesc), "r"(idesc_pv), "r"(acc0), "r"(bar_kve), "l"(qdesc), "l"(kdesc),
+          "r"(idesc_qk), "r"(bar_s_)
         : "memory");
   } else {
     asm volatile(
         "{\n\t.reg .pred e, p0, pt;\n\t.reg .b64 v1, v2, v3;\n\t.reg .b32 a1, a2, a3;\n\t"
         "elect.sync _|e, 0xffffffff;\n\t"
-        "setp.ne.b32 p0, %4, 0;\n\tsetp.eq.b32 pt, 0, 0;\n\t"
-        "add.u64 v1, %2, 128;\n\tadd.u64 v2, %2, 256;\n\tadd.u64 v3, %2, 384;\n\t"
-        "add.u32 a1, %1, 8;\n\tadd.u32 a2, %1, 32;\n\tadd.u32 a3, %1, 40;\n\t"
-        "@e tcgen05.mma.cta_group::1.kind::f16 [%0], [%1], %2, %3, p0;\n\t"
-        "@e tcgen05.mma.cta_group::1.kind::f16 [%0], [a1], v1, %3, pt;\n\t"
-        "@e tcgen05.mma.cta_group::1.kind::f16 [%0], [a2], v2, %3, pt;\n\t"
-        "@e tcgen05.mma.cta_group::1.kind::f16 [%0], [a3], v3, %3, pt;\n\t"
-        "@e tcgen05.commit.cta_group::1.mbarrier::arrive::one.shared::cluster.b64 [%5];\n\t"
-        "@e tcgen05.commit.cta_group::1.mbarrier::arrive::one.shared::cluster.b64 [%6];\n\t}"
-        ::"r"(obuf), "r"(sp), "l"(vdesc), "r"(idesc_pv), "r"(acc0), "r"(bar_kve), "r"(bar_s_)
+        "setp.ne.b32 p0, %5, 0;\n\tsetp.eq.b32 pt, 0, 0;\n\t"
+        "add.u64 v1, %3, 128;\n\tadd.u64 v2, %3, 256;\n\tadd.u64 v3, %3, 384;\n\t"
+        "add.u32 a1, %1, 8;\n\tadd.u32 a2, %2, 32;\n\tadd.u32 a3, %2, 40;\n\t"
+        "@e tcgen05.mma.cta_group::1.kind::f16 [%0], [%1], %3, %4, p0;\n\t"
+        "@e tcgen05.mma.cta_group::1.kind::f16 [%0], [a1], v1, %4, pt;\n\t"
+        "@e tcgen05.mma.cta_group::1.kind::f16 [%0], [a2], v2, %4, pt;\n\t"
+        "@e tcgen05.mma.cta_group::1.kind::f16 [%0], [a3], v3, %4, pt;\n\t"
+        "@e tcgen05.commit.cta_group::1.mbarrier::arrive::one.shared::cluster.b64 [%6];\n\t"
+        "@e tcgen05.commit.cta_group::1.mbarrier::arrive::one.shared::cluster.b64 [%7];\n\t}"
+        ::"r"(obuf), "r"(pp), "r"(sp), "l"(vdesc), "r"(idesc_pv), "r"(acc0), "r"(bar_kve), "r"(bar_s_)
         : "memory");
   }
 }
 
-__device__ __forceinline__ void lean_pv48_sep(uint32_t obuf, uint32_t pbase, uint64_t vdesc, uint32_t idesc_pv, uint32_t acc0,
-                                              uint32_t bar_kve, uint32_t bar_o_) {
-  asm volatile(
-      "{\n\t.reg .pred e, p0, pt;\n\t.reg .b64 v1, v2, v3;\n\t.reg .b32 a1, a2, a3;\n\t"
-      "elect.sync _|e, 0xffffffff;\n\t"
-      "setp.ne.b32 p0, %4, 0;\n\tsetp.eq.b32 pt, 0, 0;\n\t"
-      "add.u64 v1, %2, 128;\n\tadd.u64 v2, %2, 256;\n\tadd.u64 v3, %2, 384;\n\t"
-      "add.u32 a1, %1, 8;\n\tadd.u32 a2, %1, 16;\n\tadd.u32 a3, %1, 24;\n\t"
-      "@e tcgen05.mma.cta_group::1.kind::f16 [%0], [%1], %2, %3, p0;\n\t"
-      "@e tcgen05.mma.cta_group::1.kind::f16 [%0], [a1], v1, %3, pt;\n\t"
-      "@e tcgen05.mma.cta_group::1.kind::f16 [%0], [a2], v2, %3, pt;\n\t"
-      "@e tcgen05.mma.cta_group::1.kind::f16 [%0], [a3], v3, %3, pt;\n\t"
-      "@e tcgen05.commit.cta_group::1.mbarrier::arrive::one.shared::cluster.b64 [%5];\n\t"
-      "@e tcgen05.commit.cta_group::1.mbarrier::arrive::one.shared::cluster.b64 [%6];\n\t}"
-      ::"r"(obuf), "r"(pbase), "l"(vdesc), "r"(idesc_pv), "r"(acc0), "r"(bar_kve), "r"(bar_o_)
-      : "memory");
-}
-
 template <int DPAD, bool P_HILO>
-__global__ void __launch_bounds__(Cfg<DPAD, P_HILO>::THREADS, Cfg<DPAD, P_HILO>::MIN_CTAS)
+__global__ void __launch_bounds__(NUM_THREADS, Cfg<DPAD, P_HILO>::MIN_CTAS)
 attn_masked_kv_kernel(const __grid_constant__ CUtensorMap tm_q, const __grid_constant__ CUtensorMap tm_k,
                       const __grid_constant__ CUtensorMap tm_v, const KParams p) {
   using C = Cfg<DPAD, P_HILO>;
@@ -586,8 +600,7 @@
   const uint32_t bar_s = bar_base + 16, bar_p = bar_base + 32;
   const uint32_t bar_kv_full = bar_base + 48, bar_kv_empty = bar_base + 48 + 8 * C::NSTAGE;
   const uint32_t tmem_slot = bar_base + 48 + 16 * C::NSTAGE;
-  const uint32_t bar_f = bar_base + 192, bar_o = bar_base + 208;
-  static_assert(48 + 16 * C::NSTAGE + 8 <= 192, "barrier block layout");
+  static_assert(48 + 16 * C::NSTAGE + 8 <= 256, "barrier block layout");
   uint8_t* gen_base = smem_raw + (smem_base - smem_u32(smem_raw));
   float* const acc_smem = reinterpret_cast<float*>(gen_base + (sACC - smem_base));
   float* const mx_smem = reinterpret_cast<float*>(gen_base + (sMX - smem_base));
@@ -607,10 +620,6 @@
     mbar_init(bar_s + 8, 1);
     mbar_init(bar_p, NUM_SOFTMAX_WARPS / 2);
     mbar_init(bar_p + 8, NUM_SOFTMAX_WARPS / 2);
-    mbar_init(bar_f, NUM_SOFTMAX_WARPS / 2);
-    mbar_init(bar_f + 8, NUM_SOFTMAX_WARPS / 2);
-    mbar_init(bar_o, 1);
-    mbar_init(bar_o + 8, 1);
     for (int i = 0; i < C::NSTAGE; ++i) {
       mbar_init(bar_kv_full + 8 * i, 1);
       mbar_init(bar_kv_empty + 8 * i, 1);
@@ -684,7 +693,7 @@
         }
       }
     }
-  } else if (!C::SELF && warp == NUM_SOFTMAX_WARPS + 1) {
+  } else if (warp == NUM_SOFTMAX_WARPS + 1) {
     {
       const bool leader = elect_one();
       constexpr uint32_t idesc_qk = make_idesc(BN, 0);
@@ -718,7 +727,7 @@
       }
       FF_TRACE(0, 20);
       mbar_wait(bar_q, 0);
-      if constexpr (C::SEP) {
+      if constexpr (FF_LEAN_ISSUER && C::LAZY) {
         tc_fence_after();
         if (n_total > 0) { lean_wait(bar_kv_full, 0); tc_fence_after(); lean_qk48(tmem + C::TMEM_S, qdesc0, kdesc0, idesc_qk, bar_s); }
         if (n_total > 1) {
@@ -733,57 +742,19 @@
 #pragma unroll
           for (int u = 0; u < 4; ++u) {
             if (t < n_total) {
-              const int pstart = t >= pe2 ? pe2 : (t >= pe1 ? pe1 : (t >= pe0 ? pe0 : 0));
-              const uint32_t acc0 = (t - pstart < 2) ? 0u : 1u;
-              FF_TL(1, t, 0);
-              if (t + 2 < n_total) {
-                lean_wait(bar_kv_full + 8 * ((u + 2) & 3), u < 2 ? gph : gph ^ 1u);
-                lean_wait(bar_f + 8 * (u & 1), (uint32_t)((u >> 1) & 1));
-                FF_TL(1, t, 1);
-                tc_fence_after();
-                lean_qk48(tmem + C::TMEM_S + BN * (u & 1), qdesc0, kdesc0 + (uint64_t)((((u + 2) & 3) * C::SMEM_STAGE) >> 4),
-                          idesc_qk, bar_s + 8 * (u & 1));
-              }
-              FF_TL(1, t, 2);
-              lean_wait(bar_p, (uint32_t)(u & 1));
-              FF_TL(1, t, 3);
-              tc_fence_after();
-              lean_pv48_sep(tmem + C::TMEM_O + C::DPV * (u & 1), tmem + C::TMEM_P, vdesc0 + (uint64_t)((u * C::SMEM_STAGE) >> 4),
-                            idesc_pv, acc0, bar_kv_empty + 8 * u, bar_o + 8 * (u & 1));
-              FF_TL(1, t, 4);
-              ++t;
-            }
-          }
-          gph ^= 1u;
-        }
-        __syncwarp();
-      } else if constexpr (FF_LEAN_ISSUER && DPAD == 48 && !P_HILO && C::NSTAGE == 4) {
-        tc_fence_after();
-        if (n_total > 0) { lean_wait(bar_kv_full, 0); tc_fence_after(); lean_qk48(tmem + C::TMEM_S, qdesc0, kdesc0, idesc_qk, bar_s); }
-        if (n_total > 1) {
-          lean_wait(bar_kv_full + 8, 0);
-          tc_fence_after();
-          lean_qk48(tmem + C::TMEM_S + BN, qdesc0, kdesc0 + (uint64_t)(C::SMEM_STAGE >> 4), idesc_qk, bar_s + 8);
-        }
-        uint32_t gph = 0;
-        int t = 0;
-#pragma unroll 1
-        while (t < n_total) {
-#pragma unroll
-          for (int u = 0; u < 4; ++u) {
-            if (t < n_total) {
               const bool more = t + 2 < n_total;
               const int pstart = t >= pe2 ? pe2 : (t >= pe1 ? pe1 : (t >= pe0 ? pe0 : 0));
               const uint32_t acc0 = (t - pstart < 2) ? 0u : 1u;
               const uint32_t sp = tmem + C::TMEM_S + BN * (u & 1);
+              const uint32_t pp = tmem + C::TMEM_P + (BN / 4) * (u & 1);
               const uint32_t obuf = tmem + C::TMEM_O + C::DPV * (u & 1);
               const uint64_t vd = vdesc0 + (uint64_t)((u * C::SMEM_STAGE) >> 4);
               const uint64_t kd = kdesc0 + (uint64_t)((((u + 2) & 3) * C::SMEM_STAGE) >> 4);
               if (more) lean_wait(bar_kv_full + 8 * ((u + 2) & 3), u < 2 ? gph : gph ^ 1u);
               lean_wait(bar_p + 8 * (u & 1), (uint32_t)((u >> 1) & 1));
               tc_fence_after();
-              if (more) lean_pv_qk48<true>(obuf, sp, vd, idesc_pv, acc0, bar_kv_empty + 8 * u, qdesc0, kd, idesc_qk, bar_s + 8 * (u & 1));
-              else lean_pv_qk48<false>(obuf, sp, vd, idesc_pv, acc0, bar_kv_empty + 8 * u, 0, 0, 0, bar_s + 8 * (u & 1));
+              if (more) lean_pv_qk48<true>(obuf, pp, sp, vd, idesc_pv, acc0, bar_kv_empty + 8 * u, qdesc0, kd, idesc_qk, bar_s + 8 * (u & 1));
+              else lean_pv_qk48<false>(obuf, pp, sp, vd, idesc_pv, acc0, bar_kv_empty + 8 * u, 0, 0, 0, bar_s + 8 * (u & 1));
               ++t;
             }
           }
@@ -824,6 +795,7 @@
         const bool first_of_parity = t - pstart < 2;
         const uint64_t vd = vdesc0 + ((p_stage * (uint32_t)C::SMEM_STAGE) >> 4);
         const uint32_t pbase = tmem + C::TMEM_S + BN * (t & 1);
+        const uint32_t pslot = tmem + C::TMEM_P + (BN / 4) * (t & 1);
         const uint32_t obuf = tmem + C::TMEM_O + C::DPV * (t & 1);
         bool kv_ready = more && __all_sync(0xffffffffu, mbar_test(bar_kv_full + 8 * q_stage, q_phase));
         FF_TL(1, t, 0);
@@ -839,7 +811,7 @@
               mma_ts(obuf, pbase + 16 * ks, vdesc, idesc_pv, (!first_of_parity || ks > 0) ? 1u : 0u);
               mma_ts(obuf, pbase + 16 * ks + 8, vdesc, idesc_pv, 1u);
             } else {
-              mma_ts(obuf, pbase + 32 * (ks >> 1) + 8 * (ks & 1), vdesc, idesc_pv,
+              mma_ts(obuf, (C::LAZY && ks < 2) ? pslot + 8 * ks : pbase + 32 * (ks >> 1) + 8 * (ks & 1), vdesc, idesc_pv,
                      (!first_of_parity || ks > 0) ? 1u : 0u);
             }
           }
@@ -870,44 +842,10 @@
     const uint32_t tS = tlane + C::TMEM_S + BN * wg;
     const uint32_t tO = tlane + C::TMEM_O + C::DPV * wg;
     const uint32_t tOx = tlane + C::TMEM_O + C::DPV * (wg ^ 1);
+    const uint32_t tP = tlane + C::TMEM_P + (BN / 4) * wg;
     float* const acc_row = acc_smem + (size_t)rloc * C::ACC_LD;
     bool acc_started = false;
     int it = 0;
-    int n_total = 0;
-    [[maybe_unused]] constexpr uint32_t s_idesc_qk = make_idesc(BN, 0);
-    [[maybe_unused]] constexpr uint32_t s_idesc_pv = make_idesc(C::DPV, 1, !P_HILO);
-    [[maybe_unused]] const uint64_t s_qdesc0 = smem_desc_sw128(sQ, 16);
-    [[maybe_unused]] const uint64_t s_kdesc0 = smem_desc_sw128(sKV, 16);
-    [[maybe_unused]] const uint64_t s_vdesc0 = smem_desc_sw128(sKV + C::NKT * KV_BYTES, KV_BYTES);
-    if constexpr (C::SELF) {
-      if (wq == 0) {
-#pragma unroll 1
-        for (int ip = 0; ip < n_pass; ++ip) {
-          const FFAttnPass ps = plan->pass[ip];
-          const PassCtx cx = make_ctx(ps, p, q0);
-          if (!cx.active) continue;
-#pragma unroll 1
-          for (int seg = 0; seg < 2; ++seg) {
-            const SegCtx sg = seg ? cx.s1 : cx.s0;
-            if (sg.kv < 0) continue;
-#pragma unroll 1
-            for (int j0 = 0; j0 < n_kv_tiles;) {
-              const int cls = tile_class(sg, j0, p), j1 = run_end(sg, j0, cls, p), jb = j0;
-              j0 = j1;
-              if (!tile_skip(cx, sg, cls, p.s_kv)) n_total += j1 - jb;
-            }
-          }
-        }
-        n_total = __shfl_sync(0xffffffffu, n_total, 0);
-        if (wg < n_total) {
-          mbar_wait(bar_q, 0);
-          lean_wait(bar_kv_full + 8 * wg, 0);
-          tc_fence_after();
-          lean_qk48(tmem + C::TMEM_S + BN * wg, s_qdesc0, s_kdesc0 + (uint64_t)((wg * C::SMEM_STAGE) >> 4), s_idesc_qk,
-                    bar_s + 8 * wg);
-        }
-      }
-    }
 #pragma unroll 1
     for (int ip = 0; ip < n_pass; ++ip) {
       const FFAttnPass ps = plan->pass[ip];
@@ -918,6 +856,7 @@
         rb = (__ldg(p.bitmasks + (size_t)ps.row_mask * p.mask_words + (row >> 5)) >> (row & 31)) & 1u;
       const bool rowflip = cx.rowxor && rb;
       float m_used = -INFINITY;
+      bool lazy_ok = false;
       int n_mine = 0, last_mine = 0;
       const int it_pass0 = it;
 #pragma unroll 1
@@ -964,166 +903,109 @@
                 if (w == 0) kb_lo = kb & valid; else kb_hi = kb & valid;
               }
             }
-            float mt, sb[32];
-            {
-              float sa[32];
-              tmem_ld32(tS, sa);
-#ifdef FF_LD_BOTH
+            bool p_done = false;
+            if (C::LAZY && lazy_ok) {
+              const float nb = (cls == TILE_MIX || row_ok_cls) ? -m_used : -INFINITY;
+              uint32_t pk[16];
+              uint32_t pm;
+              {
+                float sa[32];
+                tmem_ld32(tS, sa);
+                tmem_wait_ld32(sa);
+                exp32_f16(sa, pk, cls == TILE_MIX, kb_lo, sc, nb);
+                pm = pmax16(pk);
+                tmem_st16(tP, *reinterpret_cast<const uint32_t(*)[16]>(pk));
+              }
+              {
+                float sb[32];
+                tmem_ld32(tS + 32, sb);
+                tmem_wait_ld32(sb);
+                exp32_f16(sb, pk, cls == TILE_MIX, kb_hi, sc, nb);
+                pm = max(pm, pmax16(pk));
+              }
+              if (!__any_sync(0xffffffffu, pm >= 0x5800u)) {
+                tmem_st16(tS + 32, *reinterpret_cast<const uint32_t(*)[16]>(pk));
+                p_done = true;
+              } else {
+                tmem_wait_st();
+              }
+            }
+            if (!p_done) {
+              float mt, sb[32];
+              {
+                float sa[32];
+                tmem_ld32(tS, sa);
+                tmem_wait_ld32(sa);
+                mt = max32(sa, cls == TILE_MIX, kb_lo);
+              }
               tmem_ld32(tS + 32, sb);
-#endif
-              tmem_wait_ld32(sa);
-              float m0, m1;
-              if (cls != TILE_MIX) {
-                m0 = fmaxf(sa[0], sa[1]);
-                m1 = fmaxf(sa[2], sa[3]);
-#pragma unroll
-                for (int i = 4; i < 32; i += 4) {
-                  m0 = fmaxf(m0, fmaxf(sa[i], sa[i + 1]));
-                  m1 = fmaxf(m1, fmaxf(sa[i + 2], sa[i + 3]));
-                }
-              } else {
-                m0 = m1 = -INFINITY;
-#pragma unroll
-                for (int i = 0; i < 32; i += 2) {
-                  m0 = fmaxf(m0, (kb_lo >> i) & 1u ? sa[i] : -INFINITY);
-                  m1 = fmaxf(m1, (kb_lo >> (i + 1)) & 1u ? sa[i + 1] : -INFINITY);
+              tmem_wait_ld32(sb);
+              mt = fmaxf(mt, max32(sb, cls == TILE_MIX, kb_hi));
+              if (cls != TILE_MIX && !row_ok_cls) mt = -INFINITY;
+              FF_TL(0, itj, 2);
+              const float mts = uniform ? 0.f : mt * p.scale_log2;
+              float alpha = 1.f;
+              bool grow = false;
+              if (n_mine == 0) {
+                m_used = mts;
+              } else if (mts > m_used + rescale_threshold<P_HILO>()) {
+                alpha = fast_exp2(m_used - mts);
+                m_used = mts;
+                grow = true;
+              }
+              if constexpr (C::LAZY) lazy_ok = __all_sync(0xffffffffu, m_used > -INFINITY);
+              if (__any_sync(0xffffffffu, grow)) {
+#pragma unroll
+                for (int c = 0; c < C::DPV / 16; ++c) {
+                  float o[16];
+                  uint32_t ob[16];
+                  tmem_ld16(tO + 16 * c, o);
+                  tmem_wait_ld16(o);
+#pragma unroll
+                  for (int i = 0; i < 16; ++i) ob[i] = __float_as_uint(o[i] * alpha);
+                  tmem_st16(tO + 16 * c, ob);
                 }
               }
-              mt = fmaxf(m0, m1);
-            }
-            {
-#ifdef FF_KO_LD2
-#pragma unroll
-              for (int i = 0; i < 32; ++i) sb[i] = mt + (float)i;
-#else
-#ifndef FF_LD_BOTH
-              tmem_ld32(tS + 32, sb);
-#endif
-              tmem_wait_ld32(sb);
-#endif
-              float m0, m1;
-              if (cls != TILE_MIX) {
-                m0 = fmaxf(sb[0], sb[1]);
-                m1 = fmaxf(sb[2], sb[3]);
-#pragma unroll
-                for (int i = 4; i < 32; i += 4) {
-                  m0 = fmaxf(m0, fmaxf(sb[i], sb[i + 1]));
-                  m1 = fmaxf(m1, fmaxf(sb[i + 2], sb[i + 3]));
+              FF_TL(0, itj, 3);
+              const float nb = (cls == TILE_MIX || row_ok_cls) ? -m_used : -INFINITY;
+              uint32_t pk[P_HILO ? 32 : 16];
+#pragma unroll
+              for (int hb = 1; hb >= 0; --hb) {
+                float sa[32];
+                if (hb == 0) {
+                  tmem_ld32(tS, sa);
+                  tmem_wait_ld32(sa);
                 }
-              } else {
-                m0 = m1 = -INFINITY;
-#pragma unroll
-                for (int i = 0; i < 32; i += 2) {
-                  m0 = fmaxf(m0, (kb_hi >> i) & 1u ? sb[i] : -INFINITY);
-                  m1 = fmaxf(m1, (kb_hi >> (i + 1)) & 1u ? sb[i + 1] : -INFINITY);
+                const float* sv = hb ? sb : sa;
+                const uint32_t kbits = hb ? kb_hi : kb_lo;
+                if (cls != TILE_MIX) {
+#pragma unroll
+                  for (int jj = 0; jj < 2; ++jj) {
+                    if constexpr (P_HILO) softmax_chunk_hilo<false>(sv + 16 * jj, pk + 16 * jj, sc, nb, 0u);
+                    else softmax_chunk_f16<false>(sv + 16 * jj, pk + 8 * jj, sc, nb, 0u);
+                  }
+                } else {
+#pragma unroll
+                  for (int jj = 0; jj < 2; ++jj) {
+                    const uint32_t bits = (kbits >> (16 * jj)) & 0xffffu;
+                    if constexpr (P_HILO) softmax_chunk_hilo<true>(sv + 16 * jj, pk + 16 * jj, sc, nb, bits);
+                    else softmax_chunk_f16<true>(sv + 16 * jj, pk + 8 * jj, sc, nb, bits);
+                  }
+                }
+                if constexpr (P_HILO) {
+                  tmem_st16(tS + 32 * hb, *reinterpret_cast<const uint32_t(*)[16]>(pk));
+                  tmem_st16(tS + 32 * hb + 16, *reinterpret_cast<const uint32_t(*)[16]>(pk + 16));
+                } else {
+                  tmem_st16(C::LAZY && hb == 0 ? tP : tS + 32 * hb, *reinterpret_cast<const uint32_t(*)[16]>(pk));
                 }
               }
-              mt = fmaxf(mt, fmaxf(m0, m1));
-              if (cls != TILE_MIX && !row_ok_cls) mt = -INFINITY;
-#ifdef FF_KO_MAX
-              mt = 0.f;
-#endif
-            }
-            FF_TL(0, itj, 2);
-            const float mts = uniform ? 0.f : mt * p.scale_log2;
-            float alpha = 1.f;
-            bool grow = false;
-            if (n_mine == 0) {
-              m_used = mts;
-            } else if (mts > m_used + rescale_threshold<P_HILO>()) {
-              alpha = fast_exp2(m_used - mts);
-              m_used = mts;
-              grow = true;
-            }
-            const bool any_grow = __any_sync(0xffffffffu, grow);
-            auto rescale_o = [&]() {
-#pragma unroll
-              for (int c = 0; c < C::DPV / 16; ++c) {
-                float o[16];
-                uint32_t ob[16];
-                tmem_ld16(tO + 16 * c, o);
-                tmem_wait_ld16(o);
-#pragma unroll
-                for (int i = 0; i < 16; ++i) ob[i] = __float_as_uint(o[i] * alpha);
-                tmem_st16(tO + 16 * c, ob);
-              }
-            };
-            if (!C::SEP && any_grow) rescale_o();
-            FF_TL(0, itj, 3);
-            const float nb = (cls == TILE_MIX || row_ok_cls) ? -m_used : -INFINITY;
-            uint32_t pk[(P_HILO || C::SEP) ? 32 : 16];
-#pragma unroll
-            for (int hb = 1; hb >= 0; --hb) {
-              float sa[32];
-#ifdef FF_KO_REREAD
-              const float* sv = sb;
-#else
-              if (hb == 0) {
-                tmem_ld32(tS, sa);
-                tmem_wait_ld32(sa);
-                if constexpr (C::SEP) {
-                  tc_fence_before();
-                  __syncwarp();
-                  if (lane == 0) mbar_arrive(bar_f + 8 * wg);
-                }
-              }
-              const float* sv = hb ? sb : sa;
-#endif
-              const uint32_t kbits = hb ? kb_hi : kb_lo;
-              if (cls != TILE_MIX) {
-#pragma unroll
-                for (int jj = 0; jj < 2; ++jj) {
-                  if constexpr (P_HILO) softmax_chunk_hilo<false>(sv + 16 * jj, pk + 16 * jj, sc, nb, 0u);
-                  else softmax_chunk_f16<false>(sv + 16 * jj, pk + (C::SEP ? 16 * hb : 0) + 8 * jj, sc, nb, 0u);
-                }
-              } else {
-#pragma unroll
-                for (int jj = 0; jj < 2; ++jj) {
-                  const uint32_t bits = (kbits >> (16 * jj)) & 0xffffu;
-                  if constexpr (P_HILO) softmax_chunk_hilo<true>(sv + 16 * jj, pk + 16 * jj, sc, nb, bits);
-                  else softmax_chunk_f16<true>(sv + 16 * jj, pk + (C::SEP ? 16 * hb : 0) + 8 * jj, sc, nb, bits);
-                }
-              }
-              if constexpr (P_HILO) {
-                tmem_st16(tS + 32 * hb, *reinterpret_cast<const uint32_t(*)[16]>(pk));
-                tmem_st16(tS + 32 * hb + 16, *reinterpret_cast<const uint32_t(*)[16]>(pk + 16));
-              } else if constexpr (!C::SEP) {
-                tmem_st16(tS + 32 * hb, *reinterpret_cast<const uint32_t(*)[16]>(pk));
-              }
-            }
-            if constexpr (C::SEP) {
-              if (itj >= 1) {
-                const uint32_t bo = bar_o + 8 * (wg ^ 1), po = (uint32_t)(((itj - 1) >> 1) & 1);
-                if (!mbar_test(bo, po)) mbar_wait(bo, po);
-              }
-              tc_fence_after();
-              if (any_grow) rescale_o();
-              tmem_st16(tlane + C::TMEM_P, *reinterpret_cast<const uint32_t(*)[16]>(pk));
-              tmem_st16(tlane + C::TMEM_P + 16, *reinterpret_cast<const uint32_t(*)[16]>(pk + 16));
             }
             FF_TL(0, itj, 4);
             tmem_wait_st();
             FF_TL(0, itj, 5);
             tc_fence_before();
-            if constexpr (C::SELF) {
-              named_bar_sync(3 + wg, 128);
-              if (wq == 0) {
-                const int stg = itj & 3, nxt = (itj + 2) & 3;
-                const bool more = itj + 2 < n_total;
-                if (more) lean_wait(bar_kv_full + 8 * nxt, (uint32_t)(((itj + 2) >> 2) & 1));
-                tc_fence_after();
-                const uint32_t sp = tmem + C::TMEM_S + BN * wg;
-                const uint32_t obuf = tmem + C::TMEM_O + C::DPV * wg;
-                const uint64_t vd = s_vdesc0 + (uint64_t)((stg * C::SMEM_STAGE) >> 4);
-                const uint64_t kd = s_kdesc0 + (uint64_t)((nxt * C::SMEM_STAGE) >> 4);
-                const uint32_t acc0 = n_mine == 0 ? 0u : 1u;
-                if (more) lean_pv_qk48<true>(obuf, sp, vd, s_idesc_pv, acc0, bar_kv_empty + 8 * stg, s_qdesc0, kd, s_idesc_qk, bar_s + 8 * wg);
-                else lean_pv_qk48<false>(obuf, sp, vd, s_idesc_pv, acc0, bar_kv_empty + 8 * stg, 0, 0, 0, bar_s + 8 * wg);
-              }
-            } else {
-              __syncwarp();
-              if (lane == 0) mbar_arrive(C::SEP ? bar_p : bar_p + 8 * wg);
-            }
+            __syncwarp();
+            if (lane == 0) mbar_arrive(bar_p + 8 * wg);
             FF_TL(0, itj, 6);
             FF_TRACE(itj, 34);
             ++n_mine;
@@ -1133,11 +1015,7 @@
       }
       if (it == it_pass0) continue;
       FF_TRACE(it, 35);
-      if constexpr (C::SEP) {
-        const int L = it - 1;
-        mbar_wait(bar_o + 8 * (L & 1), (uint32_t)((L >> 1) & 1));
-        tc_fence_after();
-      } else if (n_mine > 0) mbar_wait_hot<0>(bar_s + 8 * wg, ((last_mine + 2) >> 1) & 1);
+      if (n_mine > 0) mbar_wait_hot<0>(bar_s + 8 * wg, ((last_mine + 2) >> 1) & 1);
       FF_TRACE(it, 36);
       mx_smem[wg * BM + rloc] = n_mine > 0 ? m_used : -INFINITY;
       tc_fence_before();
@@ -1281,7 +1159,7 @@
   int rc = ensure_smem(attn_masked_kv_kernel<DPAD, HILO>, C::SMEM_BYTES, configured);
   if (rc != FF_OK) return rc;
   dim3 grid((kp.s_q + BM - 1) / BM, kp.heads, n_streams);
-  attn_masked_kv_kernel<DPAD, HILO><<<grid, C::THREADS, C::SMEM_BYTES, st>>>(mq, mk, mv, kp);
+  attn_masked_kv_kernel<DPAD, HILO><<<grid, NUM_THREADS, C::SMEM_BYTES, st>>>(mq, mk, mv, kp);
   return ff::check_launch("ff_attn_masked_kv");
 }
 
```
